# cebarker1000/heatflow

Hardware: AMD Instinct MI355X
Metric: DOF-updates/s (timesteps/s x nDOF) on geballe_with_diamond (higher is better)
Workload: dtype f64

## Files before the change

heatflow_amd/csrc/heatflow_hip.hip:

```cpp

#include "hf_amg_io.hpp"

namespace {

struct MeshTables {
  std::vector<int32_t> rowptr, colidx;
  ColDict spmv;
  RowGather rg;
  std::vector<char> tag_used;
  int max_blk_nnz = 0;
};

constexpr char BLOB_MAGIC[8] = {'H', 'F', 'P', 'A', 'T', '0', '2', 0};
struct BlobHeader {
  char magic[8];
  int64_t total_bytes, nnz;
  int32_t n, ne, rba, ts, max_blk_nnz, tab_len, rg_ok, rg_max_dict, spmv_max_dict, reserved;
  int64_t count[12];
};

void steady_swap(hf_ctx* ctx) {
  hf_ctx::Steady& S = ctx->steady;
  std::swap(ctx->nbc, S.nbc); std::swap(ctx->d_bc_dofs, S.bc_dofs); std::swap(ctx->d_g, S.g);
  std::swap(ctx->nlift_rows, S.nlift_rows); std::swap(ctx->nlift, S.nlift);
  std::swap(ctx->d_lift_rows, S.lift_rows); std::swap(ctx->d_lift_ptr, S.lift_ptr); std::swap(ctx->d_lift_bc, S.lift_bc);
  std::swap(ctx->d_lift_slot, S.lift_slot); std::swap(ctx->d_lift_val, S.lift_val);
  std::swap(ctx->d_A, S.K); std::swap(ctx->d_dinv, S.dinv);
  std::swap(ctx->amg, S.amg); std::swap(ctx->d_coarse_inv, S.coarse_inv); std::swap(ctx->d_coarse_inv_f, S.coarse_inv_f);
  std::swap(ctx->coarse_n, S.coarse_n); std::swap(ctx->coarse_ld, S.coarse_ld); std::swap(ctx->amg_ready, S.amg_ready);
  std::swap(ctx->amg_fine_stale, S.amg_fine_stale); std::swap(ctx->amg_opc, S.amg_opc); std::swap(ctx->amg_setup_s, S.amg_setup_s);
  std::swap(ctx->amg_print, S.amg_print);
}
struct SteadyScope {
  hf_ctx* c;
  explicit SteadyScope(hf_ctx* ctx) : c(ctx) { steady_swap(c); }
  ~SteadyScope() { steady_swap(c); }
  SteadyScope(const SteadyScope&) = delete;
  SteadyScope& operator=(const SteadyScope&) = delete;
};

void steady_free(hf_ctx* ctx) {
  {
    SteadyScope sw(ctx);
    free_amg(ctx);
  }
  hf_ctx::Steady& S = ctx->steady;
  dev_free(&S.bc_dofs); dev_free(&S.g); dev_free(&S.lift_rows); dev_free(&S.lift_ptr); dev_free(&S.lift_bc);
  dev_free(&S.lift_slot); dev_free(&S.lift_val); dev_free(&S.K); dev_free(&S.dinv); dev_free(&S.Kfree);
  dev_free(&S.hdr0); dev_free(&S.xprev); dev_free(&S.change);
  S.picard = false;
  S.nbc = S.nlift_rows = S.nlift = 0;
  S.ready = false;
  S.pred_iters = 0;
}

void load_free(hf_ctx* ctx) {
  dev_free(&ctx->d_load);
  ctx->have_load = false;
}

void tangent_free(hf_ctx* ctx) {
  free_batch_state(ctx->tanb);
  dev_free(&ctx->tan.col); dev_free(&ctx->tan.F);
  ctx->tan = hf_ctx::Tangent();
}

void kt_free(hf_ctx* ctx) {
  hf_ctx::KappaT& K = ctx->kt;
  dev_free(&K.hdr); dev_free(&K.vals); dev_free(&K.pic); dev_free(&K.b0); dev_free(&K.change);
  dev_free(&K.chdr); dev_free(&K.cvals); dev_free(&K.w);
  K = hf_ctx::KappaT();
}

void an_free(hf_ctx* ctx) {
  dev_free(&ctx->an.d_m);
  ctx->an = hf_ctx::Aniso();
}

const char* kt_kind(const hf_ctx* ctx) { return ctx->kt.k_on || !ctx->kt.c_on ? "kappa(T)" : "rho_c(T)"; }

int install_mesh(hf_ctx* ctx, int32_t n, int32_t ne, const double* zr, const int32_t* tri, const int32_t* tag, MeshTables& T) {
  free_batch(ctx);
  free_batch_state(ctx->fluxb);
  free_batch_cols(ctx);
  proj_free(ctx);
  steady_free(ctx);
  load_free(ctx);
  tangent_free(ctx);
  kt_free(ctx);
  an_free(ctx);
  ctx->n = n; ctx->ne = ne; ctx->nnz = static_cast<int64_t>(T.colidx.size());
  ctx->nchunks = (n + RB - 1) / RB;
  ctx->nblk_a = (n + RBA - 1) / RBA;
  ctx->P = std::min(ctx->nchunks, MAXP);
  if (ctx->P >= 64) ctx->P &= ~7;
  ctx->nchunks_s = (n + SRPC - 1) / SRPC;
  ctx->Ps = std::min(ctx->nchunks_s, MAXP);
  if (ctx->Ps >= 64) ctx->Ps &= ~7;
  ctx->max_chunk_nnz_s = 0;
  for (int c = 0; c < ctx->nchunks_s; ++c)
    ctx->max_chunk_nnz_s = std::max(ctx->max_chunk_nnz_s, T.rowptr[std::min<int64_t>(n, (c + 1LL) * SRPC)] - T.rowptr[static_cast<size_t>(c) * SRPC]);
  ctx->max_cdict = T.spmv.max_dict;
  ctx->c16 = true;
  if (const char* e = std::getenv("HEATFLOW_SPMV_C16")) ctx->c16 = (e[0] != '0');
  if (static_cast<size_t>(ctx->max_chunk_nnz_s + ctx->max_cdict) * 8 > 64 * 1024) ctx->c16 = false;
  ctx->cdict_own = static_cast<int>(T.spmv.ptr.size()) == ctx->nchunks_s + 1;
  for (int c = 0; c < ctx->nchunks_s && ctx->cdict_own; ++c) {
    const int32_t r0 = c * SRPC, r1 = std::min<int32_t>(n, r0 + SRPC);
    const int32_t* lo = T.spmv.dict.data() + T.spmv.ptr[c];
    const int32_t* hi = T.spmv.dict.data() + T.spmv.ptr[c + 1];
    const int32_t* at = std::lower_bound(lo, hi, r0);
    ctx->cdict_own = hi - at >= r1 - r0 && at[0] == r0 && at[r1 - r0 - 1] == r1 - 1;
  }
  ctx->max_blk_nnz = T.max_blk_nnz;
  if (static_cast<size_t>((ctx->max_blk_nnz + 1) & ~1) * 16 + (RBA + 1) * 4 > 160 * 1024)
    return fail(ctx, HF_ERR_ARG, "row block holds %d nonzeros: LDS slab too large", ctx->max_blk_nnz);
  ctx->tab_len = static_cast<int>(T.tag_used.size());
  ctx->h_tag_used = T.tag_used;
  ctx->assembled = false; ctx->have_mat = false;
  ctx->h_tri.assign(tri, tri + 3 * static_cast<size_t>(ne));
  ctx->h_tag.assign(tag, tag + ne);
  ctx->owner_ready = false;
  ctx->ncolors = 0; ctx->elist_len = 0;
  dev_free(&ctx->d_blk_eptr); dev_free(&ctx->d_blk_cptr); dev_free(&ctx->d_blk_ent);

  std::vector<int4> elem(ne);
  for (int32_t e = 0; e < ne; ++e) elem[e] = make_int4(tri[3 * e], tri[3 * e + 1], tri[3 * e + 2], tag[e]);
  HF_TRY(dev_alloc(ctx, &ctx->d_zr, n));
  HF_TRY(dev_alloc(ctx, &ctx->d_elem, ne));
  HF_TRY(dev_alloc(ctx, &ctx->d_kappa, ctx->tab_len));
  HF_TRY(dev_alloc(ctx, &ctx->d_rhoc, ctx->tab_len));
  HF_TRY(dev_alloc(ctx, &ctx->d_rowptr, n + 1));
  HF_TRY(dev_alloc(ctx, &ctx->d_colidx, ctx->nnz));
  HF_TRY(dev_alloc(ctx, &ctx->d_cdict_ptr, T.spmv.ptr.size()));
  HF_TRY(dev_alloc(ctx, &ctx->d_cdict, T.spmv.dict.size()));
  HF_TRY(dev_alloc(ctx, &ctx->d_cid, T.spmv.id.size()));
  ctx->n_cdict = static_cast<int64_t>(T.spmv.dict.size());
  HF_HIP(copy_sync(ctx, ctx->d_zr, zr, sizeof(double) * 2 * n, hipMemcpyHostToDevice));
  ctx->rg_ok = T.rg.ok && rowgather_smem_bytes(T.max_blk_nnz, T.rg.cols.max_dict) <= 160 * 1024;
  std::fill_n(ctx->rg_grid, static_cast<int>(RG_VARIANTS), 0);
  if (ctx->rg_ok) {
    const RowGather& G = T.rg;
    ctx->rg_max_dict = G.cols.max_dict;
    ctx->h_rg_tags = G.tags;
    ctx->n_rg_ell = static_cast<int64_t>(G.ell.size());
    ctx->n_rg_dict = static_cast<int64_t>(G.cols.dict.size());
    HF_TRY(dev_alloc(ctx, &ctx->d_rg_hdr, G.hdr.size()));
    HF_TRY(dev_alloc(ctx, &ctx->d_rg_ell, G.ell.size()));
    HF_TRY(dev_alloc(ctx, &ctx->d_rg_cid, G.cols.id.size() + 16));
    HF_TRY(dev_alloc(ctx, &ctx->d_rg_dict, G.cols.dict.size()));
    HF_TRY(dev_alloc(ctx, &ctx->d_rg_zrb, G.cols.dict.size()));
    HF_TRY(dev_alloc(ctx, &ctx->d_kappa_rg, 64));
    HF_TRY(dev_alloc(ctx, &ctx->d_rhoc_rg, 64));
    HF_HIP(copy_sync(ctx, ctx->d_rg_hdr, G.hdr.data(), sizeof(int4) * G.hdr.size(), hipMemcpyHostToDevice));
    HF_HIP(copy_sync(ctx, ctx->d_rg_ell, G.ell.data(), sizeof(uint16_t) * G.ell.size(), hipMemcpyHostToDevice));
    HF_HIP(hipMemsetAsync(ctx->d_rg_cid + G.cols.id.size(), 0, sizeof(uint16_t) * 16, ctx->stream));
    HF_HIP(copy_sync(ctx, ctx->d_rg_cid, G.cols.id.data(), sizeof(uint16_t) * G.cols.id.size(), hipMemcpyHostToDevice));
    HF_HIP(copy_sync(ctx, ctx->d_rg_dict, G.cols.dict.data(), sizeof(int32_t) * G.cols.dict.size(), hipMemcpyHostToDevice));
    const int64_t total = ctx->n_rg_dict;
    hipLaunchKernelGGL(k_gather_coords, dim3(static_cast<unsigned>((total + 255) / 256)), dim3(256), 0, ctx->stream, total, ctx->d_rg_dict,
                       ctx->d_zr, ctx->d_rg_zrb);
    HF_HIP(hipGetLastError());
  }
  HF_TRY(dev_alloc(ctx, &ctx->d_M, ctx->nnz));
  HF_TRY(dev_alloc(ctx, &ctx->d_A, ctx->nnz));
  HF_TRY(dev_alloc(ctx, &ctx->d_dinv, n));
  HF_TRY(dev_alloc(ctx, &ctx->d_u, n));
  HF_TRY(dev_alloc(ctx, &ctx->d_uprev, n));
  HF_TRY(dev_alloc(ctx, &ctx->d_ustart, n));
  ctx->have_prev = false;
  ctx->bdf_hist = false;
  free_responses(ctx);
  HF_TRY(dev_alloc(ctx, &ctx->d_b, n));
// ... 291 lines not shown
    HF_HIP(hipGetLastError());
    std::swap(ctx->batch, ctx->fluxnb);
    const int rc = batch_dispatch(ctx, [&](auto ops) { return decltype(ops)::pcg(ctx, false, rtol, 0.0, max_it); });
    int itmax = 0;
    for (int j = 0; j < nv; ++j) itmax = std::max(itmax, ctx->batch.h_scal[j].iters);
    std::swap(ctx->batch, ctx->fluxnb);
    if (it_out) it_out[done] = itmax;
    if (rc != HF_OK) { if (second) std::swap(F.u, F.uprev); return rc; }
    double* o = out + static_cast<size_t>(done) * nv * nfs;
    const int thr = nfs * nv;
    switch (nv) {
      case 2: hipLaunchKernelGGL((kb_gather<2>), dim3((thr + 255) / 256), dim3(256), 0, ctx->stream, nfs, ctx->d_fsamp_idx, F.u, o); break;
      case 4: hipLaunchKernelGGL((kb_gather<4>), dim3((thr + 255) / 256), dim3(256), 0, ctx->stream, nfs, ctx->d_fsamp_idx, F.u, o); break;
      case 8: hipLaunchKernelGGL((kb_gather<8>), dim3((thr + 255) / 256), dim3(256), 0, ctx->stream, nfs, ctx->d_fsamp_idx, F.u, o); break;
      default: hipLaunchKernelGGL((kb_gather<16>), dim3((thr + 255) / 256), dim3(256), 0, ctx->stream, nfs, ctx->d_fsamp_idx, F.u, o); break;
    }
    HF_HIP(hipGetLastError());
    if (second) std::swap(F.u, F.uprev);
    ++done;
  }
  return HF_OK;
}
int tangent_reset(hf_ctx* ctx) {
  hf_ctx::Batch& T = ctx->tanb;
  if (T.nv == 0) return HF_OK;
  HF_HIP(hipMemsetAsync(T.u, 0, sizeof(double) * static_cast<size_t>(ctx->n) * T.nv, ctx->stream));
  HF_HIP(hipStreamSynchronize(ctx->stream));
  T.bdf_hist = false;
  for (bool& u_ : T.pused) u_ = false;
  T.pnext = 0; T.ppending = -1;
  T.pred_iters = 0;
  return HF_OK;
}

int tangent_levels(hf_ctx* ctx) {
  hf_ctx::Batch& T = ctx->tanb;
  std::vector<int64_t> sig;
  if (ctx->precond == 1 && ctx->amg_ready)
    for (const DevLevel& L : ctx->amg) { sig.push_back(L.n); sig.push_back(L.P.ncol); }
  if (sig == ctx->tan.lev_sig) return HF_OK;
  for (auto& L : T.lev) { dev_free(&L.x); dev_free(&L.cat); if (L.own_b) dev_free(&L.b); }
  T.lev.clear();
  HF_TRY(batch_levels(ctx, T, T.nv));
  HF_HIP(hipStreamSynchronize(ctx->stream));
  ctx->tan.lev_sig = sig;
  return HF_OK;
}

int tangent_load(hf_ctx* ctx) {
  const int capd = ctx->rg_max_dict;
  const size_t sm = static_cast<size_t>(capd) * 16 + static_cast<size_t>(capd + (capd & 1)) * 8 + (RBA + 4) * 4 +
                    (static_cast<size_t>((ctx->max_blk_nnz + 1) & ~1) / 8 + 3) * 16;
  const int grid = std::min(ctx->nblk_a, 2048);
#define HF_TL(NV) hipLaunchKernelGGL(k_tangent_load<NV>, dim3(grid), dim3(RBA), sm, ctx->stream, ctx->nblk_a, capd, ctx->d_rg_hdr, \
                                     reinterpret_cast<const uint4*>(ctx->d_rg_ell), reinterpret_cast<const uint4*>(ctx->d_rg_cid), \
                                     ctx->d_rg_zrb, ctx->d_rg_dict, ctx->d_rowptr, ctx->tan.col, ctx->d_u, ctx->tan.F)
  switch (ctx->tan.nv) {
    case 2: HF_TL(2); break;
    case 4: HF_TL(4); break;
    case 8: HF_TL(8); break;
    default: HF_TL(16); break;
  }
#undef HF_TL
  HF_HIP(hipGetLastError());
  return HF_OK;
}

}

extern "C" {

const char* hf_version(void) { return "heatflow_hip 0.1 (gfx950)"; }

const char* hf_last_error(const hf_ctx* ctx) { return ctx ? ctx->err.c_str() : "null context"; }

int hf_create(int device_id, hf_ctx** out) {
  if (!out) return HF_ERR_ARG;
  *out = nullptr;
  int count = 0;
  if (hipGetDeviceCount(&count) != hipSuccess || count <= 0) return HF_ERR_HIP;
  if (device_id < 0 || device_id >= count) return HF_ERR_ARG;
  hf_ctx* ctx = new hf_ctx();
  ctx->dev = device_id;
  auto bail = [&](int rc) { *out = ctx; return rc; };
  if (hipSetDevice(device_id) != hipSuccess) return bail(fail(ctx, HF_ERR_HIP, "hipSetDevice(%d) failed", device_id));
  if (hipStreamCreateWithFlags(&ctx->stream, hipStreamNonBlocking) != hipSuccess)
    return bail(fail(ctx, HF_ERR_HIP, "hipStreamCreate failed"));
  if (hipEventCreate(&ctx->ev0) != hipSuccess || hipEventCreate(&ctx->ev1) != hipSuccess)
    return bail(fail(ctx, HF_ERR_HIP, "hipEventCreate failed"));
  if (hipHostMalloc(reinterpret_cast<void**>(&ctx->h_scal), sizeof(Scal)) != hipSuccess)
    return bail(fail(ctx, HF_ERR_ALLOC, "hipHostMalloc failed"));
  if (hipHostMalloc(reinterpret_cast<void**>(&ctx->h_mirror), sizeof(ScalMirror), hipHostMallocMapped | hipHostMallocCoherent) != hipSuccess ||
      hipHostGetDevicePointer(reinterpret_cast<void**>(&ctx->d_mirror), ctx->h_mirror, 0) != hipSuccess)
    return bail(fail(ctx, HF_ERR_ALLOC, "hipHostMalloc (mapped) failed"));
  *ctx->h_mirror = ScalMirror{};
  int rc = dev_alloc(ctx, &ctx->d_scal, 1);
  if (rc == HF_OK) rc = dev_alloc(ctx, &ctx->d_part_pAp, MAXP);
  if (rc == HF_OK) rc = dev_alloc(ctx, &ctx->d_part_rz, 2 * MAXP);
  if (rc == HF_OK) rc = dev_alloc(ctx, &ctx->d_part_zz, MAXP);
  if (rc == HF_OK) rc = dev_alloc(ctx, &ctx->d_part_bn, MAXP);
  if (rc == HF_OK && reset_scal(ctx) != HF_OK) rc = HF_ERR_HIP;
  if (rc == HF_OK) {
    hipLaunchKernelGGL(k_zero_entries, dim3(1), dim3(64), 0, ctx->stream, 0, static_cast<const int32_t*>(nullptr), static_cast<double*>(nullptr));
    if (hipStreamSynchronize(ctx->stream) != hipSuccess) rc = fail(ctx, HF_ERR_HIP, "first kernel launch failed: %s", hipGetErrorString(hipGetLastError()));
  }
  *out = ctx;
  return rc;
}

int hf_destroy(hf_ctx* ctx) {
  if (!ctx) return HF_ERR_ARG;
  (void)hipSetDevice(ctx->dev);
  if (ctx->stream) (void)hipStreamSynchronize(ctx->stream);
  dev_free(&ctx->d_zr); dev_free(&ctx->d_elem); dev_free(&ctx->d_kappa); dev_free(&ctx->d_rhoc);
  dev_free(&ctx->d_rowptr); dev_free(&ctx->d_colidx); dev_free(&ctx->d_cdict_ptr); dev_free(&ctx->d_cdict); dev_free(&ctx->d_cid); dev_free(&ctx->d_blk_eptr); dev_free(&ctx->d_blk_cptr); dev_free(&ctx->d_blk_ent); dev_free(&ctx->d_rg_hdr); dev_free(&ctx->d_rg_ell); dev_free(&ctx->d_rg_cid); dev_free(&ctx->d_rg_dict); dev_free(&ctx->d_rg_zrb); dev_free(&ctx->d_kappa_rg); dev_free(&ctx->d_rhoc_rg); dev_free(&ctx->d_M); dev_free(&ctx->d_A); dev_free(&ctx->d_dinv);
  dev_free(&ctx->d_bc_dofs); dev_free(&ctx->d_g); dev_free(&ctx->d_lift_rows); dev_free(&ctx->d_lift_ptr);
  dev_free(&ctx->d_lift_bc); dev_free(&ctx->d_lift_slot); dev_free(&ctx->d_lift_val);
  dev_free(&ctx->d_uprev); dev_free(&ctx->d_ustart);
  dev_free(&ctx->d_u); dev_free(&ctx->d_b); dev_free(&ctx->d_r); dev_free(&ctx->d_p); dev_free(&ctx->d_Ap);
  free_batch(ctx); free_batch_state(ctx->fluxb); free_batch_cols(ctx); free_amg(ctx); free_responses(ctx); proj_free(ctx); dev_free(&ctx->d_z); dev_free(&ctx->d_z2);
  steady_free(ctx); load_free(ctx); tangent_free(ctx); kt_free(ctx); an_free(ctx);
  dev_free(&ctx->d_M1); dev_free(&ctx->d_dinv1); dev_free(&ctx->d_gz); dev_free(&ctx->d_gr); dev_free(&ctx->d_bz); dev_free(&ctx->d_br);
  dev_free(&ctx->d_tmp); dev_free(&ctx->d_part_pAp); dev_free(&ctx->d_part_rz); dev_free(&ctx->d_part_zz);
  dev_free(&ctx->d_part_bn); dev_free(&ctx->d_scal); dev_free(&ctx->d_samp_idx); dev_free(&ctx->d_samp); dev_free(&ctx->d_fsamp_idx);
  for (auto& e : ctx->prof_ev) (void)hipEventDestroy(e);
  if (ctx->h_scal) (void)hipHostFree(ctx->h_scal);
  if (ctx->h_mirror) (void)hipHostFree(ctx->h_mirror);
  if (ctx->ev0) (void)hipEventDestroy(ctx->ev0);
  if (ctx->ev1) (void)hipEventDestroy(ctx->ev1);
  if (ctx->stream) (void)hipStreamDestroy(ctx->stream);
  delete ctx;
  return HF_OK;
}

int hf_set_mesh(hf_ctx* ctx, int32_t n, int32_t ne, const double* zr, const int32_t* tri, const int32_t* tag) {
  if (!ctx) return HF_ERR_ARG;
  if (!zr || !tri || !tag || n <= 0 || ne <= 0) return fail(ctx, HF_ERR_ARG, "hf_set_mesh: null pointer or empty mesh");
  HF_HIP(hipSetDevice(ctx->dev));
  int32_t maxtag = 0;
  for (int64_t k = 0; k < 3LL * ne; ++k)
    if (tri[k] < 0 || tri[k] >= n) return fail(ctx, HF_ERR_ARG, "hf_set_mesh: triangle %lld references node %d outside [0,%d)", (long long)(k / 3), tri[k], n);
  for (int32_t e = 0; e < ne; ++e) {
    if (tag[e] < 0) return fail(ctx, HF_ERR_ARG, "hf_set_mesh: negative cell tag at cell %d", e);
    maxtag = std::max(maxtag, tag[e]);
    const double* p0 = zr + 2 * tri[3 * e], *p1 = zr + 2 * tri[3 * e + 1], *p2 = zr + 2 * tri[3 * e + 2];
    const double d = (p1[0] - p0[0]) * (p2[1] - p0[1]) - (p2[0] - p0[0]) * (p1[1] - p0[1]);
    if (!(d != 0.0)) return fail(ctx, HF_ERR_ARG, "hf_set_mesh: degenerate triangle %d", e);
  }
  const auto t0 = std::chrono::steady_clock::now();
  auto lap = [&](const char* what) {
    if (std::getenv("HEATFLOW_DEBUG")) std::fprintf(stderr, "[set_mesh] %-28s %.3f s\n", what, std::chrono::duration<double>(std::chrono::steady_clock::now() - t0).count());
  };
  lap("checked");
  MeshTables T;
  Pattern P;
  HF_TRY(build_csr(ctx, n, ne, tri, P));
  lap("+ csr pattern");
  build_rowgather(n, ne, tri, tag, P);
  lap("+ row-gather lists");
  if (!build_coldict(P.rowptr, P.colidx, n, SRPC, T.spmv)) return fail(ctx, HF_ERR_ARG, "an SpMV chunk touches more than 65535 columns (16-bit positions)");
  lap("+ spmv column lists");
  T.rowptr.swap(P.rowptr);
  T.colidx.swap(P.colidx);
  T.max_blk_nnz = P.max_blk_nnz;
  T.rg = std::move(P.rg);
  T.tag_used.assign(static_cast<size_t>(maxtag) + 1, 0);
  for (int32_t e = 0; e < ne; ++e) T.tag_used[tag[e]] = 1;
  const int rc = install_mesh(ctx, n, ne, zr, tri, tag, T);
  lap("+ installed");
  return rc;
}

int hf_set_mesh_prebuilt(hf_ctx* ctx, int32_t n, int32_t ne, const double* zr, const int32_t* tri, const int32_t* tag,
                         const void* blob, int64_t bytes) {
  if (!ctx) return HF_ERR_ARG;
  if (!zr || !tri || !tag || !blob || n <= 0 || ne <= 0 || bytes <= 0) return fail(ctx, HF_ERR_ARG, "hf_set_mesh_prebuilt: null pointer or empty mesh");
  HF_HIP(hipSetDevice(ctx->dev));
  std::vector<unsigned char> staged;
  const unsigned char* src = nullptr;
  HF_TRY(blob_on_host(ctx, blob, bytes, staged, &src));
  MeshTables T;
  HF_TRY(parse_mesh_tables(ctx, src, bytes, n, ne, T));
  return install_mesh(ctx, n, ne, zr, tri, tag, T);
}

int hf_pattern_export_size(hf_ctx* ctx, int64_t* bytes) {
  if (!ctx || !bytes) return HF_ERR_ARG;
  if (!ctx->have_mesh) return fail(ctx, HF_ERR_STATE, "hf_pattern_export_size before hf_set_mesh");
  *bytes = mesh_tables_bytes(ctx);
  return HF_OK;
}

int hf_pattern_export(hf_ctx* ctx, void* blob, int64_t bytes) {
  if (!ctx || !blob) return HF_ERR_ARG;
  if (!ctx->have_mesh) return fail(ctx, HF_ERR_STATE, "hf_pattern_export before hf_set_mesh");
  if (bytes != mesh_tables_bytes(ctx)) return fail(ctx, HF_ERR_ARG, "hf_pattern_export: buffer of %lld bytes, need %lld", (long long)bytes, (long long)mesh_tables_bytes(ctx));
  HF_HIP(hipSetDevice(ctx->dev));
  std::vector<unsigned char> host(static_cast<size_t>(bytes));
  HF_TRY(write_mesh_tables(ctx, host.data()));
  HF_HIP(hipMemcpy(blob, host.data(), static_cast<size_t>(bytes), hipMemcpyDefault));
  return HF_OK;
}

int hf_set_materials(hf_ctx* ctx, int32_t n_mat, const int32_t* tags, const double* kappa, const double* rho_c) {
// ... 49 lines not shown
    m[q] = make_double2(by_tag[2 * tg], by_tag[2 * tg + 1]);
  }
  HF_HIP(hipSetDevice(ctx->dev));
  if (!any && !ctx->an.on) return HF_OK;
  if (any) {
    if (!ctx->an.d_m) HF_TRY(dev_alloc(ctx, &ctx->an.d_m, 64));
    HF_HIP(copy_sync(ctx, ctx->an.d_m, m.data(), sizeof(double2) * 64, hipMemcpyHostToDevice));
    ctx->an.h_tag = std::move(aniso);
    ctx->an.hash = fnv1a(by_tag.data(), sizeof(double) * by_tag.size());
    ctx->an.on = true;
  } else {
    an_free(ctx);
  }
  free_batch(ctx);
  ctx->assembled = false;
  ctx->pred_iters = 0;
  ctx->steady.ready = false;
  const bool from_steady = ctx->tan.steady_state;
  tangent_free(ctx);
  ctx->tan.steady_state = from_steady;
  return HF_OK;
}

int hf_update_kappa(hf_ctx* ctx, int32_t n_mat, const int32_t* tags, const double* kappa) {
  if (!ctx) return HF_ERR_ARG;
  if (!ctx->have_mat || !ctx->assembled) return fail(ctx, HF_ERR_STATE, "hf_update_kappa needs a completed hf_assemble first");
  if (n_mat <= 0 || !tags || !kappa) return fail(ctx, HF_ERR_ARG, "hf_update_kappa: bad arguments");
  HF_HIP(hipSetDevice(ctx->dev));
  std::vector<double> tk(ctx->tab_len);
  HF_HIP(copy_sync(ctx, tk.data(), ctx->d_kappa, sizeof(double) * ctx->tab_len, hipMemcpyDeviceToHost));
  for (int32_t i = 0; i < n_mat; ++i) {
    if (tags[i] < 0 || tags[i] >= ctx->tab_len || !ctx->h_tag_used[tags[i]])
      return fail(ctx, HF_ERR_ARG, "hf_update_kappa: tag %d is not a cell tag of the mesh", tags[i]);
    if (!(kappa[i] > 0.0)) return fail(ctx, HF_ERR_ARG, "hf_update_kappa: kappa must be positive");
    if (ctx->kt.k_on && ctx->kt.tabled[tags[i]])
      return fail(ctx, HF_ERR_ARG, "hf_update_kappa: tag %d carries a kappa(T) table (hf_set_kappa_tables)", tags[i]);
  }
  for (int32_t i = 0; i < n_mat; ++i) {
    tk[tags[i]] = kappa[i];
  }
  HF_HIP(copy_sync(ctx, ctx->d_kappa, tk.data(), sizeof(double) * ctx->tab_len, hipMemcpyHostToDevice));
  HF_TRY(upload_rg_tables(ctx, tk, nullptr));
  ctx->steady.ready = false;
  return hf_assemble(ctx, ctx->dt_step, ctx->mode);
}

int hf_set_dirichlet(hf_ctx* ctx, int32_t n_bc, const int32_t* dofs) {
  if (!ctx) return HF_ERR_ARG;
  if (!ctx->have_mesh) return fail(ctx, HF_ERR_STATE, "hf_set_dirichlet before hf_set_mesh");
  if (n_bc < 0 || (n_bc > 0 && !dofs)) return fail(ctx, HF_ERR_ARG, "hf_set_dirichlet: bad arguments");
  HF_HIP(hipSetDevice(ctx->dev));
  std::vector<char> seen(ctx->n, 0);
  for (int32_t q = 0; q < n_bc; ++q) {
    if (dofs[q] < 0 || dofs[q] >= ctx->n) return fail(ctx, HF_ERR_ARG, "hf_set_dirichlet: dof %d outside [0,%d)", dofs[q], ctx->n);
    if (seen[dofs[q]]) return fail(ctx, HF_ERR_ARG, "hf_set_dirichlet: dof %d listed twice (resolve overlaps on the host)", dofs[q]);
    seen[dofs[q]] = 1;
  }
  free_batch(ctx);
  ctx->nbc = n_bc;
  HF_TRY(dev_alloc(ctx, &ctx->d_bc_dofs, n_bc));
  HF_TRY(dev_alloc(ctx, &ctx->d_g, n_bc));
  if (n_bc > 0) HF_HIP(copy_sync(ctx, ctx->d_bc_dofs, dofs, sizeof(int32_t) * n_bc, hipMemcpyHostToDevice));
  HF_TRY(build_lift(ctx));
  free_amg(ctx);
  free_responses(ctx);
  ctx->assembled = false;
  return HF_OK;
}

int hf_assemble(hf_ctx* ctx, double dt, int32_t mode) {
  if (!ctx) return HF_ERR_ARG;
  if (!ctx->have_mesh || !ctx->have_mat) return fail(ctx, HF_ERR_STATE, "hf_assemble needs hf_set_mesh and hf_set_materials first");
  if (!(dt > 0.0)) return fail(ctx, HF_ERR_ARG, "hf_assemble: dt must be positive");
  if (mode < 0 || mode > 3) return fail(ctx, HF_ERR_ARG, "hf_assemble: unknown mode %d", mode);
  if (ctx->kt.on && mode != HF_ASM_ROW_GATHER)
    return fail(ctx, HF_ERR_ARG, "hf_assemble: %s tables are evaluated by the row-gather kernel only (HF_ASM_ROW_GATHER)", kt_kind(ctx));
  if (ctx->an.on && (mode != HF_ASM_ROW_GATHER || !ctx->rg_ok))
    return fail(ctx, HF_ERR_ARG, "hf_assemble: anisotropic conductivities (hf_set_anisotropy) are assembled by the row-gather kernel only (HF_ASM_ROW_GATHER)");
  HF_HIP(hipSetDevice(ctx->dev));
  ctx->dt_step = dt;
  ctx->dt = ctx->scheme == HF_TIME_BDF2 ? 2.0 * dt / 3.0 : dt;
  ctx->mode = mode;
  HF_HIP(hipEventRecord(ctx->ev0, ctx->stream));
  HF_TRY(launch_assemble(ctx));
  if (ctx->kt.on) {
    HF_TRY(kt_revalue(ctx, ctx->d_u, nullptr));
  } else {
    if (ctx->nbc > 0) {
      if (ctx->nlift > 0)
        hipLaunchKernelGGL(k_take_lift, dim3((ctx->nlift + 255) / 256), dim3(256), 0, ctx->stream, ctx->nlift,
                           ctx->d_lift_slot, ctx->d_A, ctx->d_lift_val);
      hipLaunchKernelGGL(k_bc_rows, dim3((ctx->nbc + 255) / 256), dim3(256), 0, ctx->stream, ctx->nbc, ctx->d_bc_dofs,
                         ctx->d_rowptr, ctx->d_colidx, ctx->d_A);
    }
    hipLaunchKernelGGL(k_dinv, dim3((ctx->n + 255) / 256), dim3(256), 0, ctx->stream, ctx->n, ctx->d_rowptr,
                       ctx->d_colidx, ctx->d_A, ctx->d_dinv);
  }
  HF_HIP(hipEventRecord(ctx->ev1, ctx->stream));
  HF_HIP(hipGetLastError());
  HF_HIP(hipStreamSynchronize(ctx->stream));
  float ms = 0.f;
  HF_HIP(hipEventElapsedTime(&ms, ctx->ev0, ctx->ev1));
  ctx->last_ms = ms;
  if (ctx->precond == 1) {
    OperatorPrint now;
    HF_TRY(operator_print(ctx, now));
    if (!(ctx->amg_ready && ctx->amg_reuse)) {
      HF_TRY(build_amg_auto(ctx));
      ctx->amg_print = std::move(now);
    } else {
      ctx->amg_fine_stale = !same_print(now, ctx->amg_print) || ctx->kt.on;
    }
  }
  if (ctx->precond == 1 && ctx->amg_ready) {
    ctx->amg[0].A.val = ctx->d_A;
    ctx->amg[0].dinv = ctx->d_dinv;
  }
  ctx->assembled = true;
  ctx->pred_iters = 0;
  ctx->have_prev = false;
  ctx->bdf_hist = false;
  free_responses(ctx);
  return tangent_reset(ctx);
}

int hf_set_precond(hf_ctx* ctx, int32_t kind, int32_t reuse) {
  if (!ctx) return HF_ERR_ARG;
  if (kind < 0 || kind > 1) return fail(ctx, HF_ERR_ARG, "hf_set_precond: unknown preconditioner %d", kind);
  if (kind != ctx->precond) { ctx->assembled = false; ctx->pred_iters = 0; (void)hipSetDevice(ctx->dev); free_batch(ctx); }
  if (kind == 0) { (void)hipSetDevice(ctx->dev); free_amg(ctx); }
  ctx->precond = kind;
  ctx->amg_reuse = reuse ? 1 : 0;
  return HF_OK;
}

int hf_set_time_scheme(hf_ctx* ctx, int32_t scheme) {
  if (!ctx) return HF_ERR_ARG;
  if (scheme != HF_TIME_BACKWARD_EULER && scheme != HF_TIME_BDF2) return fail(ctx, HF_ERR_ARG, "hf_set_time_scheme: unknown scheme %d", scheme);
  if (scheme != ctx->scheme) {
    (void)hipSetDevice(ctx->dev);
    free_batch(ctx);
    ctx->assembled = false;
    ctx->pred_iters = 0;
    ctx->scheme = scheme;
  }
  return HF_OK;
}

int kt_set_tables(hf_ctx* ctx, bool cap, int32_t n_tab, const int32_t* tags, const double* t0, const double* dT, const int32_t* n_knots,
                  const double* values) {
  const char* fn = cap ? "hf_set_rhoc_tables" : "hf_set_kappa_tables";
  const char* what = cap ? "rho_c(T)" : "kappa(T)";
  if (!ctx) return HF_ERR_ARG;
  if (!ctx->have_mesh) return fail(ctx, HF_ERR_STATE, "%s before hf_set_mesh", fn);
  if (n_tab < 0) return fail(ctx, HF_ERR_ARG, "%s: negative table count", fn);
  HF_HIP(hipSetDevice(ctx->dev));
  hf_ctx::KappaT& K = ctx->kt;
  if (n_tab == 0) {
    if (ctx->steady.picard) ctx->steady.ready = false;
    if (cap ? K.c_on : K.k_on) {
      free_batch(ctx);
      ctx->assembled = false;
      ctx->pred_iters = 0;
    }
    if (!(cap ? K.k_on : K.c_on)) { kt_free(ctx); return HF_OK; }
    if (cap ? K.c_on : K.k_on) {
      const std::vector<KTab> none(64, KTab{0.0, 0.0, 0, 0});
      HF_HIP(copy_sync(ctx, cap ? K.chdr : K.hdr, none.data(), sizeof(KTab) * 64, hipMemcpyHostToDevice));
      dev_free(cap ? &K.cvals : &K.vals);
      (cap ? K.ctabled : K.tabled).clear();
      (cap ? K.c_on : K.k_on) = false;
      K.have_change = false;
    }
    return HF_OK;
  }
  if (!tags || !t0 || !dT || !n_knots || !values) return fail(ctx, HF_ERR_ARG, "%s: null pointer", fn);
  if (ctx->an.on) return fail(ctx, HF_ERR_STATE, "%s: anisotropic conductivities are set (hf_set_anisotropy; the table kernels are isotropic)", fn);
  if (!ctx->rg_ok || (ctx->assembled && ctx->mode != HF_ASM_ROW_GATHER))
    return fail(ctx, HF_ERR_ARG, "%s: %s is evaluated by the row-gather kernel only (HF_ASM_ROW_GATHER on a mesh with row-gather lists)", fn, what);
  if (cap && ct_smem_bytes(ctx->max_blk_nnz, ctx->rg_max_dict) + 2 * 64 * sizeof(KTab) > 160 * 1024)
    return fail(ctx, HF_ERR_ARG, "%s: the (M, A) slab, the staged state and the table headers of this mesh exceed the 160 KiB of LDS", fn);
  std::vector<KTab> hdr(64, KTab{0.0, 0.0, 0, 0});
  std::vector<double> vals;
  std::vector<char> tabled(ctx->tab_len, 0);
  for (int32_t i = 0; i < n_tab; ++i) {
    const int32_t tg = tags[i];
// ... 437 lines not shown
  if (ctx->have_load) return fail(ctx, HF_ERR_STATE, "hf_run_tangent: a load is set (tangents of pre-heated runs are not supported)");
  if (!ctx->tan.ready) return fail(ctx, HF_ERR_STATE, "hf_run_tangent before hf_tangent_setup");
  if (ctx->tan.steady_state)
    return fail(ctx, HF_ERR_STATE, "hf_run_tangent: the state comes from hf_steady_solve and depends on the conductivities (tangents start at zero): hf_set_state first");
  if (!ctx->assembled) return fail(ctx, HF_ERR_STATE, "hf_run_tangent before hf_assemble");
  if (ctx->mode != HF_ASM_ROW_GATHER) return fail(ctx, HF_ERR_ARG, "hf_run_tangent: the operator was not assembled by the row-gather kernel");
  if (n_steps <= 0 || (ctx->nbc > 0 && !g_all) || max_it <= 0 || rtol < 0 || atol < 0) return fail(ctx, HF_ERR_ARG, "hf_run_tangent: bad arguments");
  if (ns < 0 || (ns > 0 && (!nodes || !samples || !tangent_samples))) return fail(ctx, HF_ERR_ARG, "hf_run_tangent: bad sample arguments");
  for (int32_t q = 0; q < ns; ++q)
    if (nodes[q] < 0 || nodes[q] >= ctx->n) return fail(ctx, HF_ERR_ARG, "hf_run_tangent: node %d outside [0,%d)", nodes[q], ctx->n);
  HF_HIP(hipSetDevice(ctx->dev));
  hf_ctx::Batch& T = ctx->tanb;
  const int nv = T.nv;
  const size_t hstep = static_cast<size_t>(ctx->nbc) * nv;
  DevTemp<double> t_gall, t_hall, t_sall, t_tall;
  if (ctx->nbc > 0) {
    HF_TRY(dev_alloc(ctx, &t_gall.p, static_cast<size_t>(n_steps) * ctx->nbc));
    HF_HIP(copy_sync(ctx, t_gall.p, g_all, sizeof(double) * n_steps * ctx->nbc, hipMemcpyHostToDevice));
    HF_TRY(dev_alloc(ctx, &t_hall.p, h_all ? hstep * n_steps : hstep));
    if (h_all) HF_HIP(copy_sync(ctx, t_hall.p, h_all, sizeof(double) * hstep * n_steps, hipMemcpyHostToDevice));
    else HF_HIP(hipMemsetAsync(t_hall.p, 0, sizeof(double) * hstep, ctx->stream));
  }
  if (ns > 0) {
    HF_TRY(ensure_samples(ctx, ns));
    HF_TRY(dev_alloc(ctx, &t_sall.p, static_cast<size_t>(n_steps) * ns));
    HF_TRY(dev_alloc(ctx, &t_tall.p, static_cast<size_t>(n_steps) * nv * ns));
    HF_HIP(copy_sync(ctx, ctx->d_samp_idx, nodes, sizeof(int32_t) * ns, hipMemcpyHostToDevice));
  }
  HF_TRY(ensure_batch_cols(ctx, nv));
  T.lds = ctx->bcols.nv == nv;
  HF_TRY(tangent_levels(ctx));
  int rc = HF_OK;
  HF_HIP(hipEventRecord(ctx->ev0, ctx->stream));
  for (int32_t s = 0; s < n_steps && rc == HF_OK; ++s) {
    rc = step_device(ctx, ctx->nbc > 0 ? g_all + static_cast<size_t>(s) * ctx->nbc : nullptr,
                     ctx->nbc > 0 ? t_gall.p + static_cast<size_t>(s) * ctx->nbc : nullptr, rtol, atol, max_it);
    if (iters) iters[s] = ctx->h_scal->iters;
    if (rc != HF_OK) break;
    if (ns > 0)
      hipLaunchKernelGGL(k_gather, dim3((ns + 255) / 256), dim3(256), 0, ctx->stream, ns, ctx->d_samp_idx, ctx->d_u,
                         t_sall.p + static_cast<size_t>(s) * ns);
    HF_TRY(tangent_load(ctx));
    const double* hs = ctx->nbc == 0 ? nullptr : t_hall.p + (h_all ? hstep * s : 0);
    std::swap(ctx->batch, ctx->tanb);
    rc = batch_dispatch(ctx, [&](auto ops) { return decltype(ops)::step(ctx, hs, rtol, atol, max_it); });
    std::swap(ctx->batch, ctx->tanb);
    if (tangent_iters)
      for (int j = 0; j < nv; ++j) tangent_iters[static_cast<size_t>(s) * nv + j] = T.h_scal[j].iters;
    if (ns > 0 && rc == HF_OK) {
      double* out = t_tall.p + static_cast<size_t>(s) * nv * ns;
      const int thr = ns * nv;
      switch (nv) {
        case 2: hipLaunchKernelGGL((kb_gather<2>), dim3((thr + 255) / 256), dim3(256), 0, ctx->stream, ns, ctx->d_samp_idx, T.u, out); break;
        case 4: hipLaunchKernelGGL((kb_gather<4>), dim3((thr + 255) / 256), dim3(256), 0, ctx->stream, ns, ctx->d_samp_idx, T.u, out); break;
        case 8: hipLaunchKernelGGL((kb_gather<8>), dim3((thr + 255) / 256), dim3(256), 0, ctx->stream, ns, ctx->d_samp_idx, T.u, out); break;
        default: hipLaunchKernelGGL((kb_gather<16>), dim3((thr + 255) / 256), dim3(256), 0, ctx->stream, ns, ctx->d_samp_idx, T.u, out); break;
      }
    }
  }
  (void)hipEventRecord(ctx->ev1, ctx->stream);
  (void)hipStreamSynchronize(ctx->stream);
  float ms = 0.f;
  (void)hipEventElapsedTime(&ms, ctx->ev0, ctx->ev1);
  ctx->last_ms = ms;
  if (ns > 0 && rc == HF_OK) {
    (void)copy_sync(ctx, samples, t_sall.p, sizeof(double) * n_steps * ns, hipMemcpyDeviceToHost);
    (void)copy_sync(ctx, tangent_samples, t_tall.p, sizeof(double) * n_steps * nv * ns, hipMemcpyDeviceToHost);
  }
  return rc;
}

int hf_get_tangent(hf_ctx* ctx, int32_t j, double* s) {
  if (!ctx) return HF_ERR_ARG;
  if (!ctx->tan.ready) return fail(ctx, HF_ERR_STATE, "hf_get_tangent before hf_tangent_setup");
  if (j < 0 || j >= ctx->tan.nv || !s) return fail(ctx, HF_ERR_ARG, "hf_get_tangent: column %d outside [0,%d) or null pointer", j, ctx->tan.nv);
  HF_HIP(hipSetDevice(ctx->dev));
  hipLaunchKernelGGL(kb_get_column, dim3(1024), dim3(256), 0, ctx->stream, static_cast<size_t>(ctx->n), ctx->tan.nv, j, ctx->tanb.u, ctx->d_tmp);
  HF_HIP(hipGetLastError());
  HF_HIP(copy_sync(ctx, s, ctx->d_tmp, sizeof(double) * ctx->n, hipMemcpyDeviceToHost));
  return HF_OK;
}

int steady_eliminate(hf_ctx* ctx) {
  HF_HIP(hipMemcpyAsync(ctx->d_A, ctx->steady.Kfree, sizeof(double) * ctx->nnz, hipMemcpyDeviceToDevice, ctx->stream));
  if (ctx->nlift > 0)
    hipLaunchKernelGGL(k_take_lift, dim3((ctx->nlift + 255) / 256), dim3(256), 0, ctx->stream, ctx->nlift, ctx->d_lift_slot,
                       ctx->d_A, ctx->d_lift_val);
  hipLaunchKernelGGL(k_bc_rows, dim3((ctx->nbc + 255) / 256), dim3(256), 0, ctx->stream, ctx->nbc, ctx->d_bc_dofs, ctx->d_rowptr,
                     ctx->d_colidx, ctx->d_A);
  hipLaunchKernelGGL(k_dinv, dim3((ctx->n + 255) / 256), dim3(256), 0, ctx->stream, ctx->n, ctx->d_rowptr, ctx->d_colidx, ctx->d_A, ctx->d_dinv);
  HF_HIP(hipGetLastError());
  return HF_OK;
}

int steady_setup_impl(hf_ctx* ctx, const char* fn, bool picard, int32_t n_s, const int32_t* dofs, int32_t precond) {
  if (n_s <= 0 || !dofs) return fail(ctx, HF_ERR_ARG, "%s: empty Dirichlet set (the stiffness alone is singular)", fn);
  if (precond < 0 || precond > 1) return fail(ctx, HF_ERR_ARG, "%s: unknown preconditioner %d", fn, precond);
  if (!ctx->rg_ok || (ctx->assembled && ctx->mode != HF_ASM_ROW_GATHER))
    return fail(ctx, HF_ERR_ARG, "%s: the steady operator is assembled by the row-gather kernel only (HF_ASM_ROW_GATHER on a mesh with row-gather lists)", fn);
  std::vector<char> seen(ctx->n, 0);
  for (int32_t q = 0; q < n_s; ++q) {
    if (dofs[q] < 0 || dofs[q] >= ctx->n) return fail(ctx, HF_ERR_ARG, "%s: dof %d outside [0,%d)", fn, dofs[q], ctx->n);
    if (seen[dofs[q]]) return fail(ctx, HF_ERR_ARG, "%s: dof %d listed twice (resolve overlaps on the host)", fn, dofs[q]);
    seen[dofs[q]] = 1;
  }
  HF_HIP(hipSetDevice(ctx->dev));
  steady_free(ctx);
  hf_ctx::Steady& S = ctx->steady;
  const int n = ctx->n;
  S.nbc = n_s;
  HF_TRY(dev_alloc(ctx, &S.bc_dofs, n_s));
  HF_TRY(dev_alloc(ctx, &S.g, n_s));
  HF_TRY(dev_alloc(ctx, &S.Kfree, ctx->nnz));
  HF_TRY(dev_alloc(ctx, &S.K, ctx->nnz));
  HF_TRY(dev_alloc(ctx, &S.dinv, n));
  if (picard) {
    HF_TRY(dev_alloc(ctx, &S.xprev, n));
    HF_TRY(dev_alloc(ctx, &S.change, 1));
    if (!ctx->kt.hdr) {
      const std::vector<KTab> none(64, KTab{0.0, 0.0, 0, 0});
      HF_TRY(dev_alloc(ctx, &S.hdr0, 64));
      HF_HIP(copy_sync(ctx, S.hdr0, none.data(), sizeof(KTab) * 64, hipMemcpyHostToDevice));
    }
  }
  HF_HIP(copy_sync(ctx, S.bc_dofs, dofs, sizeof(int32_t) * n_s, hipMemcpyHostToDevice));
  HF_HIP(hipEventRecord(ctx->ev0, ctx->stream));
  if (picard) HF_TRY(steady_revalue(ctx, ctx->kt.hdr ? ctx->kt.hdr : S.hdr0, ctx->d_u, S.Kfree));
  else HF_TRY(launch_assemble_rows_any<true>(ctx, ctx->d_kappa_rg, ctx->d_rhoc_rg, 1.0, nullptr, S.Kfree));
  {
    SteadyScope sw(ctx);
    HF_TRY(build_lift(ctx));
    HF_TRY(steady_eliminate(ctx));
    HF_HIP(hipEventRecord(ctx->ev1, ctx->stream));
    HF_HIP(hipGetLastError());
    HF_HIP(hipStreamSynchronize(ctx->stream));
    float ms = 0.f;
    HF_HIP(hipEventElapsedTime(&ms, ctx->ev0, ctx->ev1));
    ctx->last_ms = ms;
    if (precond == 1) HF_TRY(build_amg_auto(ctx));
  }
  S.precond = precond;
  S.pred_iters = 0;
  S.picard = picard;
  S.ready = true;
  return HF_OK;
}

int hf_steady_setup(hf_ctx* ctx, int32_t n_s, const int32_t* dofs, int32_t precond) {
  if (!ctx) return HF_ERR_ARG;
  if (!ctx->have_mesh || !ctx->have_mat) return fail(ctx, HF_ERR_STATE, "hf_steady_setup needs hf_set_mesh and hf_set_materials first");
  if (ctx->kt.on) return fail(ctx, HF_ERR_STATE, "hf_steady_setup: %s tables are set (a Picard steady state is not supported)", kt_kind(ctx));
  return steady_setup_impl(ctx, "hf_steady_setup", false, n_s, dofs, precond);
}

int hf_steady_picard_setup(hf_ctx* ctx, int32_t n_s, const int32_t* dofs, int32_t precond) {
  if (!ctx) return HF_ERR_ARG;
  if (!ctx->have_mesh || !ctx->have_mat) return fail(ctx, HF_ERR_STATE, "hf_steady_picard_setup needs hf_set_mesh and hf_set_materials first");
  if (ctx->an.on)
    return fail(ctx, HF_ERR_STATE, "hf_steady_picard_setup: anisotropic conductivities are set (hf_set_anisotropy; the table kernels are isotropic)");
  return steady_setup_impl(ctx, "hf_steady_picard_setup", true, n_s, dofs, precond);
}

int hf_steady_picard_solve(hf_ctx* ctx, const double* g_s, int32_t use_load, double rtol, double atol, int32_t max_it, double picard_tol,
                           int32_t max_sweeps, int32_t* sweeps, int32_t* iters, double* change, double* nl_resid) {
  if (!ctx) return HF_ERR_ARG;
  if (!ctx->steady.ready || !ctx->steady.picard)
// ... 341 lines not shown
  for (int32_t q = 0; q < ns; ++q)
    if (nodes[q] < 0 || nodes[q] >= ctx->n) return fail(ctx, HF_ERR_ARG, "hf_batch_run: node %d outside [0,%d)", nodes[q], ctx->n);
  const int ncomp = (flux_components & 1) + ((flux_components >> 1) & 1);
  if (flux_components != 0) {
    if (flux_components < 0 || flux_components > 3 || flux_max_it <= 0 || flux_rtol < 0 || nfs <= 0 || !flux_nodes || !flux_samples)
      return fail(ctx, HF_ERR_ARG, "hf_batch_run_flux: bad flux arguments");
    if (!ctx->flux_ready) return fail(ctx, HF_ERR_STATE, "hf_batch_run_flux before hf_flux_setup");
    if (!ctx->rg_ok) return fail(ctx, HF_ERR_ARG, "hf_batch_run_flux: the row-gather lists are not available for this mesh (a row of more than 32 entries or more than 64 cell tags): project run by run");
    for (int32_t q = 0; q < nfs; ++q)
      if (flux_nodes[q] < 0 || flux_nodes[q] >= ctx->n) return fail(ctx, HF_ERR_ARG, "hf_batch_run_flux: node %d outside [0,%d)", flux_nodes[q], ctx->n);
  }
  HF_HIP(hipSetDevice(ctx->dev));
  const int nv = B.nv;
  const size_t gstep = static_cast<size_t>(ctx->nbc) * nv;
  DevTemp<double> t_sall, t_fall;
  if (flux_components != 0) {
    HF_TRY(ensure_batch_flux(ctx, nv, ncomp));
    if (nfs > ctx->fsamp_cap) { HF_TRY(dev_alloc(ctx, &ctx->d_fsamp_idx, nfs)); ctx->fsamp_cap = nfs; }
    HF_HIP(copy_sync(ctx, ctx->d_fsamp_idx, flux_nodes, sizeof(int32_t) * nfs, hipMemcpyHostToDevice));
    HF_TRY(dev_alloc(ctx, &t_fall.p, static_cast<size_t>(n_steps) * ncomp * nv * nfs));
  }
  if (ctx->nbc > 0) {
    HF_TRY(dev_alloc(ctx, &B.g, gstep * n_steps));
    HF_HIP(copy_sync(ctx, B.g, g_all, sizeof(double) * gstep * n_steps, hipMemcpyHostToDevice));
  }
  if (ns > 0) {
    HF_TRY(ensure_samples(ctx, ns));
    HF_TRY(dev_alloc(ctx, &t_sall.p, static_cast<size_t>(n_steps) * nv * ns));
    HF_HIP(copy_sync(ctx, ctx->d_samp_idx, nodes, sizeof(int32_t) * ns, hipMemcpyHostToDevice));
  }
  int rc = HF_OK;
  HF_HIP(hipEventRecord(ctx->ev0, ctx->stream));
  for (int32_t s = 0; s < n_steps && rc == HF_OK; ++s) {
    const double* gs = ctx->nbc > 0 ? B.g + gstep * s : nullptr;
    rc = batch_dispatch(ctx, [&](auto ops) { return decltype(ops)::step(ctx, gs, rtol, atol, max_it); });
    if (iters)
      for (int j = 0; j < nv; ++j) iters[static_cast<size_t>(s) * nv + j] = B.h_scal[j].iters;
    if (ns > 0 && rc == HF_OK) {
      double* out = t_sall.p + static_cast<size_t>(s) * nv * ns;
      const int thr = ns * nv;
      switch (nv) {
        case 2: hipLaunchKernelGGL((kb_gather<2>), dim3((thr + 255) / 256), dim3(256), 0, ctx->stream, ns, ctx->d_samp_idx, B.u, out); break;
        case 4: hipLaunchKernelGGL((kb_gather<4>), dim3((thr + 255) / 256), dim3(256), 0, ctx->stream, ns, ctx->d_samp_idx, B.u, out); break;
        case 8: hipLaunchKernelGGL((kb_gather<8>), dim3((thr + 255) / 256), dim3(256), 0, ctx->stream, ns, ctx->d_samp_idx, B.u, out); break;
        default: hipLaunchKernelGGL((kb_gather<16>), dim3((thr + 255) / 256), dim3(256), 0, ctx->stream, ns, ctx->d_samp_idx, B.u, out); break;
      }
    }
    if (flux_components != 0 && rc == HF_OK)
      rc = batch_flux_step(ctx, flux_components, flux_rtol, flux_max_it, nfs, t_fall.p + static_cast<size_t>(s) * ncomp * nv * nfs,
                           flux_iters ? flux_iters + static_cast<size_t>(s) * ncomp : nullptr);
  }
  (void)hipEventRecord(ctx->ev1, ctx->stream);
  (void)hipStreamSynchronize(ctx->stream);
  float ms = 0.f;
  (void)hipEventElapsedTime(&ms, ctx->ev0, ctx->ev1);
  ctx->last_ms = ms;
  if (ns > 0 && rc == HF_OK) (void)copy_sync(ctx, samples, t_sall.p, sizeof(double) * n_steps * nv * ns, hipMemcpyDeviceToHost);
  if (flux_components != 0 && rc == HF_OK)
    (void)copy_sync(ctx, flux_samples, t_fall.p, sizeof(double) * n_steps * ncomp * nv * nfs, hipMemcpyDeviceToHost);
  return rc;
}

int hf_get_sizes(hf_ctx* ctx, int32_t* n, int32_t* ne, int64_t* nnz, int32_t* nbc) {
  if (!ctx) return HF_ERR_ARG;
  if (n) *n = ctx->n;
  if (ne) *ne = ctx->ne;
  if (nnz) *nnz = ctx->nnz;
  if (nbc) *nbc = ctx->nbc;
  return HF_OK;
}

int hf_get_csr(hf_ctx* ctx, int32_t* rowptr, int32_t* colidx, double* A, double* M) {
  if (!ctx) return HF_ERR_ARG;
  if (!ctx->have_mesh) return fail(ctx, HF_ERR_STATE, "hf_get_csr before hf_set_mesh");
  if ((A || M) && !ctx->assembled) return fail(ctx, HF_ERR_STATE, "hf_get_csr: values requested before hf_assemble");
  HF_HIP(hipSetDevice(ctx->dev));
  if (rowptr) std::memcpy(rowptr, ctx->h_rowptr.data(), sizeof(int32_t) * (ctx->n + 1));
  if (colidx) std::memcpy(colidx, ctx->h_colidx.data(), sizeof(int32_t) * ctx->nnz);
  if (A) HF_HIP(copy_sync(ctx, A, ctx->d_A, sizeof(double) * ctx->nnz, hipMemcpyDeviceToHost));
  if (M) HF_HIP(copy_sync(ctx, M, ctx->d_M, sizeof(double) * ctx->nnz, hipMemcpyDeviceToHost));
  return HF_OK;
}

int hf_spmv(hf_ctx* ctx, int32_t which, const double* x, double* y) {
  if (!ctx) return HF_ERR_ARG;
  if (!ctx->assembled || !x || !y || which < 0 || which > 1) return fail(ctx, HF_ERR_STATE, "hf_spmv: not assembled or bad arguments");
  HF_HIP(hipSetDevice(ctx->dev));
  HF_HIP(copy_sync(ctx, ctx->d_tmp, x, sizeof(double) * ctx->n, hipMemcpyHostToDevice));
  launch_spmv<0>(ctx, which ? ctx->d_M : ctx->d_A, ctx->d_tmp, ctx->d_Ap);
  HF_HIP(hipGetLastError());
  HF_HIP(hipStreamSynchronize(ctx->stream));
  HF_HIP(copy_sync(ctx, y, ctx->d_Ap, sizeof(double) * ctx->n, hipMemcpyDeviceToHost));
  return HF_OK;
}

int hf_amg_apply(hf_ctx* ctx, const double* r, double* z, double* rz) {
  if (!ctx || !r || !z) return HF_ERR_ARG;
  if (ctx->precond != 1 || !ctx->amg_ready || !ctx->assembled || ctx->amg.empty())
    return fail(ctx, HF_ERR_STATE, "hf_amg_apply: no assembled operator with a multigrid hierarchy (hf_set_precond(1, ...) and hf_assemble first)");
  HF_HIP(hipSetDevice(ctx->dev));
  const int n = ctx->n, nl = static_cast<int>(ctx->amg.size());
  HF_TRY(reset_scal(ctx));
  std::vector<double> dinv(n), z0(n);
  HF_HIP(copy_sync(ctx, dinv.data(), ctx->d_dinv, sizeof(double) * n, hipMemcpyDeviceToHost));
  const double w0 = ctx->amg[0].omega;
  for (int i = 0; i < n; ++i) z0[i] = w0 * (dinv[i] * r[i]);
  auto poison = [&](double* p, size_t count) { return count ? hipMemsetAsync(p, 0xFF, sizeof(double) * count, ctx->stream) : hipSuccess; };
  HF_HIP(poison(ctx->d_tmp, n));
  HF_HIP(poison(ctx->d_z2, n));
  HF_HIP(poison(ctx->d_part_rz, MAXP));
  for (int l = 1; l < nl; ++l) {
    DevLevel& L = ctx->amg[l];
    if (L.cat) HF_HIP(poison(L.cat, static_cast<size_t>(L.n) + ctx->amg[l + 1].n));
    else HF_HIP(poison(L.b, L.n));
    if (l == 1) HF_HIP(poison(L.res, L.n));
  }
  HF_HIP(copy_sync(ctx, ctx->d_r, r, sizeof(double) * n, hipMemcpyHostToDevice));
  HF_HIP(copy_sync(ctx, ctx->d_z, z0.data(), sizeof(double) * n, hipMemcpyHostToDevice));
  vcycle(ctx, 0);
  HF_HIP(hipGetLastError());
  HF_HIP(hipStreamSynchronize(ctx->stream));
  HF_HIP(copy_sync(ctx, z, ctx->d_z2, sizeof(double) * n, hipMemcpyDeviceToHost));
  if (rz) {
    std::vector<double> part(ctx->P);
    HF_HIP(copy_sync(ctx, part.data(), ctx->d_part_rz, sizeof(double) * ctx->P, hipMemcpyDeviceToHost));
    double s = 0.0;
    for (double v : part) s += v;
    *rz = s;
  }
  return HF_OK;
}

int hf_batch_apply_precond(hf_ctx* ctx, const double* r, double* z, double* rz) {
  if (!ctx || !r || !z) return HF_ERR_ARG;
  hf_ctx::Batch& B = ctx->batch;
  if (B.nv == 0) return fail(ctx, HF_ERR_STATE, "hf_batch_apply_precond: no batch is open (hf_batch_begin)");
  if (ctx->precond != 1 || !ctx->amg_ready || !ctx->assembled || ctx->amg.empty() || B.lev.size() != ctx->amg.size())
    return fail(ctx, HF_ERR_STATE, "hf_batch_apply_precond: the batch has no multigrid hierarchy");
  HF_HIP(hipSetDevice(ctx->dev));
  const int nv = B.nv, nl = static_cast<int>(ctx->amg.size());
  const size_t n = static_cast<size_t>(ctx->n), vec = n * nv;
  const bool dpc = B.opk != HF_BATCH_SHARED;
  std::vector<double> dinv(dpc ? vec : n), ri(vec), z0(vec);
  HF_HIP(copy_sync(ctx, dinv.data(), dpc ? B.dinv : ctx->d_dinv, sizeof(double) * dinv.size(), hipMemcpyDeviceToHost));
  const double w0 = ctx->amg[0].omega;
  for (size_t i = 0; i < n; ++i)
    for (int j = 0; j < nv; ++j) {
      const size_t q = i * nv + j;
      ri[q] = r[static_cast<size_t>(j) * n + i];
      z0[q] = w0 * ((dpc ? dinv[q] : dinv[i]) * ri[q]);
    }
  auto poison = [&](double* p, size_t count) { return count ? hipMemsetAsync(p, 0xFF, sizeof(double) * count, ctx->stream) : hipSuccess; };
  HF_HIP(poison(B.tmp, vec));
  HF_HIP(poison(B.z2, vec));
  HF_HIP(poison(B.part_rz, static_cast<size_t>(nv) * MAXP));
  for (int l = 1; l < nl; ++l) {
    const hf_ctx::BatchLevel& Q = B.lev[l];
    const size_t ln = static_cast<size_t>(ctx->amg[l].n);
    if (Q.cat) HF_HIP(poison(Q.cat, (ln + ctx->amg[l + 1].n) * nv));
    else HF_HIP(poison(Q.b, ln * nv));
    if (l == 1) HF_HIP(poison(Q.res, ln * nv));
  }
  HF_HIP(hipMemsetAsync(B.scal, 0, sizeof(Scal) * nv, ctx->stream));
  HF_HIP(copy_sync(ctx, B.r, ri.data(), sizeof(double) * vec, hipMemcpyHostToDevice));
  HF_HIP(copy_sync(ctx, B.z, z0.data(), sizeof(double) * vec, hipMemcpyHostToDevice));
  HF_TRY(batch_dispatch(ctx, [&](auto ops) { decltype(ops)::vcycle(ctx, 0); return HF_OK; }));
// ... 151 lines not shown
```

heatflow_amd/csrc/hf_context.hpp:

```cpp

#pragma once
#include <hip/hip_runtime.h>
#include <hip/hip_ext.h>

#include <algorithm>
#include <chrono>
#include <cmath>
#include <cstdarg>
#include <cstdint>
#include <cstdio>
#include <cstdlib>
#include <cstring>
#include <string>
#include <thread>
#include <vector>

#include "amg_host.hpp"
#include "heatflow_hip.h"

namespace {

constexpr int RB = 256;
#ifndef HF_RBA
#define HF_RBA 256
#endif
constexpr int RBA = HF_RBA;
constexpr int TPB = 256;
constexpr int NCOL = 32;
#ifndef HF_STAGE_U
#define HF_STAGE_U 2
#endif
#ifndef HF_UNROLL
#define HF_UNROLL 4
#endif
constexpr int MAXP = 1024;
constexpr int MAXRESP = 4;
#ifndef HF_PROJ_MH
#define HF_PROJ_MH 6
#endif
constexpr int PROJ_MH = HF_PROJ_MH;
constexpr int PROJ_MT = PROJ_MH + MAXRESP;
constexpr int TS = 512;
#ifndef HF_SPMV_RPC
#define HF_SPMV_RPC 512
#endif
#ifndef HF_SPMV_UN
#define HF_SPMV_UN 8
#endif
constexpr int SRPC = HF_SPMV_RPC;

struct ScalMirror {
  double zz, bn2;
  int iters;
  int pad_;
  unsigned long long done_st;
  unsigned long long tested_st;
};
inline int mirror_tested(const ScalMirror* m, unsigned epoch) {
  const unsigned long long v = __atomic_load_n(&m->tested_st, __ATOMIC_ACQUIRE);
  return static_cast<unsigned>(v >> 32) == epoch ? static_cast<int>(v & 0xffffffffu) - 1 : -1;
}
inline int mirror_done(const ScalMirror* m, unsigned epoch) {
  const unsigned long long v = __atomic_load_n(&m->done_st, __ATOMIC_ACQUIRE);
  return static_cast<unsigned>(v >> 32) == epoch ? static_cast<int>(v & 0xffffffffu) : 0;
}

struct Scal {
  double tol2;
  double bn2;
  double zz;
  int iters;
  int done;
  int first;
  unsigned epoch;
  ScalMirror* mirror;
};

constexpr int NV_MAX = 16;
struct BRed { double pAp[NV_MAX], rz[2][NV_MAX], zz[NV_MAX], bn[NV_MAX]; };

constexpr int KT_MAX_KNOTS = 256;
constexpr int KT_MAX_PICARD = 8;
struct KTab { double t0, inv_dt; int n, off; };

enum RgVariant { RG_ROWS, RG_ROWS_K, RG_AN, RG_AN_K, RG_KT, RG_CT, RG_KT_K, RG_VARIANTS };

}

struct hf_ctx {
  int dev = 0;
  hipStream_t stream = nullptr;
  hipEvent_t ev0 = nullptr, ev1 = nullptr;
  std::string err;
  double last_ms = 0.0;

  int32_t n = 0, ne = 0, nbc = 0;
  int64_t nnz = 0;
  int nchunks = 0, P = 0;
  int nchunks_s = 0, Ps = 0;
  int max_chunk_nnz_s = 0;
  int32_t *d_cdict_ptr = nullptr, *d_cdict = nullptr;
  uint16_t* d_cid = nullptr;
  int max_cdict = 0;
  bool cdict_own = false;
  bool c16 = true;
  bool have_mesh = false, have_mat = false, assembled = false;
  double dt = 0.0;
  double dt_step = 0.0;
  int mode = 0;
  int scheme = HF_TIME_BACKWARD_EULER;

  std::vector<int32_t> h_rowptr, h_colidx, h_tri, h_tag;
  std::vector<char> h_tag_used;
  bool owner_ready = false;

  double2* d_zr = nullptr;
  int4* d_elem = nullptr;
  int tab_len = 0;
  double *d_kappa = nullptr, *d_rhoc = nullptr;
  int32_t *d_rowptr = nullptr, *d_colidx = nullptr;
  int32_t *d_blk_eptr = nullptr, *d_blk_cptr = nullptr;
  int2* d_blk_ent = nullptr;
  int nblk_a = 0;
  int max_blk_nnz = 0, ncolors = 0;
  int64_t elist_len = 0;
  bool rg_ok = false;
  int4* d_rg_hdr = nullptr;
  uint16_t *d_rg_ell = nullptr, *d_rg_cid = nullptr;
  int32_t* d_rg_dict = nullptr;
  double2* d_rg_zrb = nullptr;
  int rg_max_dict = 0;
  int rg_grid[RG_VARIANTS] = {};
  int64_t n_rg_ell = 0, n_rg_dict = 0, n_cdict = 0;
  std::vector<int32_t> h_rg_tags;
  double *d_kappa_rg = nullptr, *d_rhoc_rg = nullptr;
  struct Aniso {
    bool on = false;
    double2* d_m = nullptr;
    std::vector<char> h_tag;
    uint64_t hash = 0;
  } an;
  double *d_M = nullptr, *d_A = nullptr, *d_dinv = nullptr;
  int32_t* d_bc_dofs = nullptr;
  double* d_g = nullptr;
  int32_t nlift_rows = 0, nlift = 0;
  int32_t *d_lift_rows = nullptr, *d_lift_ptr = nullptr, *d_lift_bc = nullptr, *d_lift_slot = nullptr;
  double* d_lift_val = nullptr;
  double *d_u = nullptr, *d_b = nullptr, *d_r = nullptr, *d_p = nullptr, *d_Ap = nullptr;
  double *d_uprev = nullptr, *d_ustart = nullptr;
  bool have_prev = false;
  bool bdf_hist = false;
  int extrapolate = 1;
  int start_kind = 3;
  std::vector<double> h_g0, h_g1;
  int g_hist = 0;
  struct BcResponse { std::vector<double> dir; double* w = nullptr; };
  std::vector<BcResponse> resp;
  long long resp_solves = 0;
  struct Proj {
    double *V[PROJ_MT] = {nullptr}, *F[PROJ_MT] = {nullptr};
    bool used[PROJ_MT] = {false};
    int next = 0, pending = -1;
    double *G = nullptr, *alpha = nullptr, *part = nullptr;
    bool ready = false;
  } proj;
  double *d_tmp = nullptr;
  double *d_part_pAp = nullptr, *d_part_rz = nullptr, *d_part_zz = nullptr, *d_part_bn = nullptr;
  Scal* d_scal = nullptr;
  Scal* h_scal = nullptr;
  ScalMirror* h_mirror = nullptr;
  ScalMirror* d_mirror = nullptr;
  unsigned epoch = 0;
  int32_t* d_samp_idx = nullptr;
  double* d_samp = nullptr;
  int samp_cap = 0;
  int pred_iters = 0;
  int precond = 0;
  int amg_reuse = 0;
  bool amg_ready = false;
  struct DevCsr {
    int nrow = 0, ncol = 0, lanes = 8; int64_t nnz = 0; int32_t *ptr = nullptr, *idx = nullptr; double* val = nullptr;
    float* valf = nullptr;
    int max_row = 0;
    int rpc = 0, nchunks = 0, chunk_nnz = 0;
    int32_t *dptr = nullptr, *dict = nullptr;
    uint16_t* cid = nullptr;
    int max_dict = 0;
    int64_t ndict = 0;
// ... 173 lines not shown
```

heatflow_amd/csrc/hf_kernels.hpp:

```cpp
#pragma once
#include <type_traits>

#include "hf_context.hpp"

namespace {


template <int NW = 4>
__device__ __forceinline__ double block_sum(double v, double* sw) {
#pragma unroll
  for (int o = 32; o > 0; o >>= 1) v += __shfl_down(v, o, 64);
  const int w = threadIdx.x >> 6;
  if ((threadIdx.x & 63) == 0) sw[w] = v;
  __syncthreads();
  double t = sw[0];
#pragma unroll
  for (int k = 1; k < NW; ++k) t += sw[k];
  __syncthreads();
  return t;
}

__device__ __forceinline__ double sum_partials(const double* __restrict__ part, int P, double* s4) {
  double v = 0.0;
  for (int k = threadIdx.x; k < P; k += TPB) v += part[k];
// ... 701 lines not shown

__global__ void k_take_lift(int nlift, const int32_t* __restrict__ slot, double* __restrict__ A,
                            double* __restrict__ val) {
  const int q = blockIdx.x * blockDim.x + threadIdx.x;
  if (q >= nlift) return;
  val[q] = A[slot[q]];
  A[slot[q]] = 0.0;
}

__global__ void k_bc_rows(int nbc, const int32_t* __restrict__ dofs, const int32_t* __restrict__ rowptr,
                          const int32_t* __restrict__ colidx, double* __restrict__ A) {
  const int q = blockIdx.x * blockDim.x + threadIdx.x;
  if (q >= nbc) return;
  const int row = dofs[q];
  for (int k = rowptr[row]; k < rowptr[row + 1]; ++k) A[k] = (colidx[k] == row) ? 1.0 : 0.0;
}

__global__ void k_dinv(int n, const int32_t* __restrict__ rowptr, const int32_t* __restrict__ colidx,
                       const double* __restrict__ A, double* __restrict__ dinv) {
  const int row = blockIdx.x * blockDim.x + threadIdx.x;
  if (row >= n) return;
  double d = 0.0;
  for (int k = rowptr[row]; k < rowptr[row + 1]; ++k)
    if (colidx[k] == row) d = A[k];
  dinv[row] = 1.0 / d;
}

__global__ void k_lift(int nrows, const int32_t* __restrict__ rows, const int32_t* __restrict__ ptr,
                       const int32_t* __restrict__ bc, const double* __restrict__ val,
                       const double* __restrict__ g, double* __restrict__ b) {
  const int q = blockIdx.x * blockDim.x + threadIdx.x;
  if (q >= nrows) return;
  double s = 0.0;
  for (int k = ptr[q]; k < ptr[q + 1]; ++k) s += val[k] * g[bc[k]];
  b[rows[q]] -= s;
}

__global__ void k_set_bc(int nbc, const int32_t* __restrict__ dofs, const double* __restrict__ g,
                         double* __restrict__ b, double* __restrict__ u) {
  const int q = blockIdx.x * blockDim.x + threadIdx.x;
  if (q >= nbc) return;
  b[dofs[q]] = g[q];
  u[dofs[q]] = g[q];
}

__global__ void k_gather(int ns, const int32_t* __restrict__ idx, const double* __restrict__ u,
                         double* __restrict__ out) {
  const int q = blockIdx.x * blockDim.x + threadIdx.x;
  if (q < ns) out[q] = u[idx[q]];
}

__global__ __launch_bounds__(TPB) void k_hold_load(int n, const int32_t* __restrict__ rowptr, const int32_t* __restrict__ colidx,
                                                   const double* __restrict__ K, const double* __restrict__ u,
                                                   const unsigned char* __restrict__ mask, double* __restrict__ F) {
  const int row = blockIdx.x * blockDim.x + threadIdx.x;
  if (row >= n) return;
  double s = 0.0;
  if (!mask[row])
    for (int k = rowptr[row]; k < rowptr[row + 1]; ++k) s += K[k] * u[colidx[k]];
  F[row] = s;
}

__global__ void k_mark_rows(int nq, const int32_t* __restrict__ idx, unsigned char* __restrict__ mask) {
  const int q = blockIdx.x * blockDim.x + threadIdx.x;
  if (q < nq) mask[idx[q]] = 1;
}

__device__ __forceinline__ unsigned long long mirror_stamp(unsigned epoch, int v) {
  return (static_cast<unsigned long long>(epoch) << 32) | static_cast<unsigned>(v);
}
__device__ __forceinline__ void mirror_publish(ScalMirror* m, double zz, int iters, int done, unsigned epoch) {
  if (m == nullptr) return;
  m->zz = zz;
  m->iters = iters;
  __hip_atomic_store(&m->done_st, mirror_stamp(epoch, done), __ATOMIC_RELAXED, __HIP_MEMORY_SCOPE_SYSTEM);
  __threadfence_system();
  __hip_atomic_store(&m->tested_st, mirror_stamp(epoch, iters + 1), __ATOMIC_RELEASE, __HIP_MEMORY_SCOPE_SYSTEM);
}
__device__ __forceinline__ void mirror_breakdown(ScalMirror* m, unsigned epoch) {
  if (m != nullptr) __hip_atomic_store(&m->done_st, mirror_stamp(epoch, 2), __ATOMIC_RELEASE, __HIP_MEMORY_SCOPE_SYSTEM);
}

struct ColComp { const int32_t* dptr; const int32_t* dict; const uint16_t* id; int xd_off; int own; };

#ifndef HF_NT_STREAM
#define HF_NT_STREAM 0
#endif
#ifndef HF_PIPE
#define HF_PIPE 1
#endif
#ifndef HF_PHASE_CLOCK
#define HF_PHASE_CLOCK -1
#endif
#if HF_PHASE_CLOCK >= 0
#ifndef HF_PHASE_CONV
#define HF_PHASE_CONV 0
#endif
__device__ unsigned long long g_phase[MAXP * 16];
#define HF_STAMP(slot)                                                                                   \
  do {                                                                                                   \
    if (MODE == HF_PHASE_CLOCK && C16 && (MODE != 0 || (part2 != nullptr) == (HF_PHASE_CONV != 0)) && threadIdx.x == 0 && (slot) < 16) \
      g_phase[blockIdx.x * 16 + (slot)] = wall_clock64();                                                \
  } while (0)
#else
#define HF_STAMP(slot) do { } while (0)
#endif
template <typename T>
__device__ __forceinline__ T stream_load(const T* p) {
#if HF_NT_STREAM
  return __builtin_nontemporal_load(p);
#else
  return *p;
#endif
}

__device__ __forceinline__ double bdf2_operand(double un, double unm1) { return (4.0 * un - unm1) * (1.0 / 3.0); }

template <int MODE, bool C16 = false, typename VT = double, int UN = 8>
__global__ __launch_bounds__(TS) __attribute__((amdgpu_waves_per_eu(8, 8))) void k_spmv(int n, int nchunks, int rpc ,
                                              const int32_t* __restrict__ rowptr, const int32_t* __restrict__ colidx,
                                              const VT* __restrict__ vals, const double* __restrict__ x,
                                              double* __restrict__ y, Scal* __restrict__ scal,
                                              double* __restrict__ part0, const double* __restrict__ bvec,
                                              const double* __restrict__ dinv, double* __restrict__ pvec,
                                              double* __restrict__ part1, double* __restrict__ part2, double w,
                                              int npart ,
                                              int parity, ColComp comp) {
  extern __shared__ double sprod[];
  __shared__ double s4[TS / 64];
  __shared__ int s_own;
  constexpr bool BDF = MODE >= 12 && MODE <= 15;
  auto opnd = [&](int c) { return BDF ? bdf2_operand(x[c], bvec[c]) : x[c]; };
  if ((MODE == 3 || MODE == 4 || MODE == 6 || MODE == 9) && scal->done) return;
  if ((MODE == 0 || MODE == 7) && scal != nullptr && scal->done) return;
  double acc0 = 0.0, acc1 = 0.0, acc2 = 0.0;
  double beta = 0.0;
  bool first9 = false;
  if (MODE == 9) {
    first9 = scal->first != 0;
    if (!first9) {
      double v0 = 0.0, v1 = 0.0, v2 = 0.0;
      for (int k = threadIdx.x; k < npart; k += TS) {
        v0 += part1[parity * MAXP + k];
        v1 += part1[(parity ^ 1) * MAXP + k];
        v2 += part2[k];
      }
      const double rz_new = block_sum<TS / 64>(v0, s4);
      const double rz_old = block_sum<TS / 64>(v1, s4);
      const double zz = block_sum<TS / 64>(v2, s4);
      const bool conv = zz <= scal->tol2;
      if (blockIdx.x == 0 && threadIdx.x == 0) {
        scal->zz = zz;
        if (conv) scal->done = 1;
      }
      if (conv) return;
      beta = rz_new / rz_old;
    }
  }
  auto cycle_gate = [&]() {
    if (!((MODE == 3 || MODE == 0) && part2 != nullptr)) return false;
    double v2 = 0.0;
    for (int k = threadIdx.x; k < npart; k += TS) v2 += part2[k];
    const double zz = block_sum<TS / 64>(v2, s4);
    const bool conv = zz <= scal->tol2;
    if (blockIdx.x == 0 && threadIdx.x == 0) {
      if (conv) { scal->zz = zz; scal->done = 1; }
      mirror_publish(scal->mirror, zz, scal->iters, conv ? 1 : 0, scal->epoch);
    }
    return conv;
  };
  constexpr bool PIPELINED = C16 && (HF_PIPE == 2 || (HF_PIPE == 1 && sizeof(VT) == 4));
  if (!PIPELINED && cycle_gate()) return;
  const ChunkIter sched(nchunks);
  HF_STAMP(0);
  int stamp_at = 1;
  (void)stamp_at;
  const int tpr = (MODE == 0 || MODE == 6 || MODE == 7) ? TS / rpc : 1;
  const int prel = static_cast<int>(threadIdx.x) / tpr;
  const int psub = static_cast<int>(threadIdx.x) % tpr;
  struct RowOps { double b, d, y, p, x; };
  auto row_operands = [&](int prc, bool from_slice) {
    RowOps e{0.0, 0.0, 0.0, 0.0, 0.0};
    if (MODE == 2 || MODE == 3 || MODE == 4 || MODE == 5 || MODE == 7 || MODE == 8 || MODE == 11 || MODE == 13 || MODE == 15) e.b = bvec[prc];
    if (MODE == 2 || MODE == 4 || MODE == 5 || MODE == 10 || MODE == 11 || MODE == 14 || MODE == 15) e.d = dinv[prc];
    if (MODE == 6 || (MODE == 9 && !first9)) e.y = y[prc];
    if (MODE == 9 && !first9) e.p = pvec[prc];
    if ((MODE == 4 || MODE == 8 || MODE == 9 || MODE == 11) && !from_slice) e.x = x[prc];
    if (BDF) e.x = x[prc];
    return e;
  };
  auto rows_phase = [&](bool pin, int prow, int pa, int pb, const RowOps& e) {
    if ((MODE == 0 || MODE == 6 || MODE == 7) && tpr > 1) {
      double s = 0.0;
      if (pin)
        for (int j = pa + psub; j < pb; j += tpr) s += sprod[j];
      for (int o = tpr >> 1; o > 0; o >>= 1) s += __shfl_down(s, o, 64);
      if (pin && psub == 0) {
        y[prow] = (MODE == 6) ? e.y + s : s;
        if (MODE == 7) acc0 += e.b * s;
      }
    } else if (pin) {
      const int row = prow;
      double s = 0.0;
      for (int j = pa; j < pb; ++j) s += sprod[j];
      if (MODE == 0) {
        y[row] = s;
      } else if (MODE == 2) {
        const double ri = e.b - s;
        const double zi = e.d * ri;
        y[row] = ri;
        pvec[row] = zi;
        acc0 += ri * zi;
        acc1 += zi * zi;
        acc2 += (e.d * e.b) * (e.d * e.b);
      } else if (MODE == 3) {
        y[row] = e.b - s;
      } else if (MODE == 4) {
        const double yi = e.x + w * e.d * (e.b - s);
        y[row] = yi;
        acc0 += e.b * yi;
      } else if (MODE == 5) {
        const double ri = e.b - s;
        y[row] = ri;
        pvec[row] = w * e.d * ri;
        acc1 += (e.d * ri) * (e.d * ri);
        acc2 += (e.d * e.b) * (e.d * e.b);
      } else if (MODE == 7) {
        y[row] = s;
        acc0 += e.b * s;
      } else if (MODE == 6) {
        y[row] = e.y + s;
      } else if (MODE == 8) {
        y[row] = s;
        pvec[row] = 2.0 * e.x - e.b;
      } else if (MODE == 10) {
        y[row] = s + w * e.d;
      } else if (MODE == 11) {
        y[row] = s + w * e.d;
        pvec[row] = 2.0 * e.x - e.b;
      } else if (BDF) {
        y[row] = (MODE == 14 || MODE == 15) ? s + w * e.d : s;
        pvec[row] = (MODE == 13 || MODE == 15) ? 2.0 * e.x - e.b : e.x;
      } else {
        const double api = first9 ? s : s + beta * e.y;
        const double pi = first9 ? e.x : e.x + beta * e.p;
        y[row] = api;
        pvec[row] = pi;
        acc0 += pi * api;
      }
    }
  };
  if (PIPELINED) {
    struct Bounds { int k0, k1, d0, d1; };
    auto bounds = [&](int ch) {
// ... 23 lines not shown
    Bounds cur = bounds(min(sched.chunk, nchunks - 1));
    heads(cur, sched.chunk < sched.end);
    if (cycle_gate()) return;
    for (int chunk = sched.chunk; chunk < sched.end; chunk += sched.step) {
      const bool more = chunk + sched.step < sched.end;
      const int r0 = chunk * rpc, r1 = min(n, r0 + rpc);
      const int k0 = cur.k0, k1 = cur.k1, d0 = cur.d0, nd = cur.d1 - cur.d0;
      const int prow = r0 + prel;
      const bool pin = prow < r1;
      const int prc = min(prow, r1 - 1);
      int c0[HF_STAGE_U];
      double x0[HF_STAGE_U];
#pragma unroll
      for (int u = 0; u < HF_STAGE_U; ++u) { c0[u] = lhead[u]; x0[u] = opnd(c0[u]); }
      const Bounds nxt = bounds(more ? chunk + sched.step : chunk);
      const int pa = rowptr[prc] - k0, pb = rowptr[prc + 1] - k0;
      RowOps e = row_operands(prc, comp.own != 0);
#pragma unroll
      for (int u = 0; u < HF_STAGE_U; ++u) {
        const int i = static_cast<int>(threadIdx.x) + u * TS;
        if (i < nd) {
          xd[i] = x0[u];
          if ((MODE == 4 || MODE == 8 || MODE == 9 || MODE == 11) && c0[u] == r0) s_own = i;
        }
      }
      for (int i = threadIdx.x + HF_STAGE_U * TS; i < nd; i += HF_STAGE_U * TS) {
        int c[HF_STAGE_U];
        double xv[HF_STAGE_U];
#pragma unroll
        for (int u = 0; u < HF_STAGE_U; ++u) c[u] = comp.dict[d0 + min(i + u * TS, nd - 1)];
#pragma unroll
        for (int u = 0; u < HF_STAGE_U; ++u) xv[u] = opnd(c[u]);
#pragma unroll
        for (int u = 0; u < HF_STAGE_U; ++u)
          if (i + u * TS < nd) {
            xd[i + u * TS] = xv[u];
            if ((MODE == 4 || MODE == 8 || MODE == 9 || MODE == 11) && c[u] == r0) s_own = i + u * TS;
          }
      }
      __syncthreads();
      HF_STAMP(stamp_at); ++stamp_at;
      if ((MODE == 4 || MODE == 8 || MODE == 9 || MODE == 11) && comp.own && pin) e.x = xd[s_own + (prow - r0)];
#pragma unroll
      for (int u = 0; u < UN; ++u) {
        const int kk = k0 + static_cast<int>(threadIdx.x) + u * TS;
        if (kk < k1) sprod[kk - k0] = v[u] * xd[id[u]];
      }
      for (int kb = k0 + UN * TS; kb < k1; kb += UN * TS) {
#pragma unroll
        for (int u = 0; u < UN; ++u) {
          const int kk = min(kb + static_cast<int>(threadIdx.x) + u * TS, k1 - 1);
          v[u] = static_cast<double>(stream_load(&vals[kk]));
          id[u] = static_cast<int>(stream_load(&comp.id[kk]));
        }
#pragma unroll
        for (int u = 0; u < UN; ++u) {
          const int kk = kb + static_cast<int>(threadIdx.x) + u * TS;
          if (kk < k1) sprod[kk - k0] = v[u] * xd[id[u]];
        }
      }
      heads(nxt, more);
      __syncthreads();
      HF_STAMP(stamp_at); ++stamp_at;
      rows_phase(pin, prow, pa, pb, e);
      __syncthreads();
      HF_STAMP(stamp_at); ++stamp_at;
      cur = nxt;
    }
  } else {
  const ChunkIter& sched_ = sched;
  for (int chunk = sched_.chunk; chunk < sched_.end; chunk += sched_.step) {
    const int r0 = chunk * rpc;
    const int r1 = min(n, r0 + rpc);
    const int k0 = rowptr[r0];
    const int k1 = rowptr[r1];
    const int prow = r0 + prel;
    const bool pin = prow < r1;
    int pa = 0, pb = 0;
    if (pin) {
      pa = rowptr[prow] - k0;
      pb = rowptr[prow + 1] - k0;
    }
    RowOps e = row_operands(min(prow, r1 - 1), C16 && comp.own != 0);
    if (C16) {
      double* xd = sprod + comp.xd_off;
      const int d0 = comp.dptr[chunk], nd = comp.dptr[chunk + 1] - d0;
      int k = k0 + threadIdx.x;
      double v[HF_UNROLL];
      int id[HF_UNROLL];
#pragma unroll
      for (int u = 0; u < HF_UNROLL; ++u) {
        const bool in = k + u * TS < k1;
        v[u] = in ? static_cast<double>(stream_load(&vals[k + u * TS])) : 0.0;
        id[u] = in ? static_cast<int>(stream_load(&comp.id[k + u * TS])) : 0;
      }
      for (int i = threadIdx.x; i < nd; i += HF_STAGE_U * TS) {
        int c[HF_STAGE_U];
        double xv[HF_STAGE_U];
#pragma unroll
        for (int u = 0; u < HF_STAGE_U; ++u) c[u] = (i + u * TS < nd) ? comp.dict[d0 + i + u * TS] : 0;
#pragma unroll
        for (int u = 0; u < HF_STAGE_U; ++u) xv[u] = (i + u * TS < nd) ? opnd(c[u]) : 0.0;
#pragma unroll
        for (int u = 0; u < HF_STAGE_U; ++u)
          if (i + u * TS < nd) {
            xd[i + u * TS] = xv[u];
            if ((MODE == 4 || MODE == 8 || MODE == 9 || MODE == 11) && c[u] == r0) s_own = i + u * TS;
          }
      }
      __syncthreads();
      HF_STAMP(stamp_at); ++stamp_at;
      if ((MODE == 4 || MODE == 8 || MODE == 9 || MODE == 11) && comp.own && pin) e.x = xd[s_own + (prow - r0)];
      while (k < k1) {
        const int kn = k + HF_UNROLL * TS;
        double vn[HF_UNROLL];
        int idn[HF_UNROLL];
#pragma unroll
        for (int u = 0; u < HF_UNROLL; ++u) {
          const bool in = kn + u * TS < k1;
          vn[u] = in ? static_cast<double>(stream_load(&vals[kn + u * TS])) : 0.0;
          idn[u] = in ? static_cast<int>(stream_load(&comp.id[kn + u * TS])) : 0;
        }
#pragma unroll
        for (int u = 0; u < HF_UNROLL; ++u)
          if (k + u * TS < k1) sprod[k - k0 + u * TS] = v[u] * xd[id[u]];
#pragma unroll
        for (int u = 0; u < HF_UNROLL; ++u) { v[u] = vn[u]; id[u] = idn[u]; }
        k = kn;
      }
    } else {
      for (int k = k0 + threadIdx.x; k < k1; k += HF_UNROLL * TS) {
        int c[HF_UNROLL];
        double v[HF_UNROLL], xv[HF_UNROLL];
#pragma unroll
        for (int u = 0; u < HF_UNROLL; ++u) {
          const bool in = k + u * TS < k1;
          c[u] = in ? colidx[k + u * TS] : 0;
          v[u] = in ? static_cast<double>(vals[k + u * TS]) : 0.0;
        }
#pragma unroll
        for (int u = 0; u < HF_UNROLL; ++u) xv[u] = (k + u * TS < k1) ? opnd(c[u]) : 0.0;
#pragma unroll
        for (int u = 0; u < HF_UNROLL; ++u)
          if (k + u * TS < k1) sprod[k - k0 + u * TS] = v[u] * xv[u];
      }
    }
    __syncthreads();
    HF_STAMP(stamp_at); ++stamp_at;
    rows_phase(pin, prow, pa, pb, e);
    __syncthreads();
    HF_STAMP(stamp_at); ++stamp_at;
  }
  }
  if (MODE == 2 || MODE == 7 || MODE == 9 || (MODE == 4 && part0 != nullptr)) {
    const double t0 = block_sum<TS / 64>(acc0, s4);
    if (threadIdx.x == 0) {
      part0[blockIdx.x] = t0;
      for (int q = blockIdx.x + gridDim.x; q < npart; q += gridDim.x) part0[q] = 0.0;
    }
  }
  if (MODE == 2 || MODE == 5) {
    const double t1 = block_sum<TS / 64>(acc1, s4);
    const double t2 = block_sum<TS / 64>(acc2, s4);
    if (threadIdx.x == 0) {
      part1[blockIdx.x] = t1;
      part2[blockIdx.x] = t2;
      for (int q = blockIdx.x + gridDim.x; q < npart; q += gridDim.x) { part1[q] = 0.0; part2[q] = 0.0; }
    }
  }
}

__global__ __launch_bounds__(TPB) void k_pcg_begin(int P, double rtol, double atol, const double* __restrict__ part_zz,
                                                   const double* __restrict__ part_bn, Scal* __restrict__ scal, unsigned epoch) {
  __shared__ double s4[4];
  const double zz = sum_partials(part_zz, P, s4);
  const double bn2 = sum_partials(part_bn, P, s4);
  if (threadIdx.x == 0) {
    const double tol = fmax(rtol * sqrt(bn2 > 0.0 ? bn2 : zz), atol);
    scal->tol2 = tol * tol;
    scal->bn2 = bn2;
    scal->zz = zz;
    scal->iters = 0;
    scal->first = 1;
    scal->done = (zz <= tol * tol) ? 1 : 0;
    scal->epoch = epoch;
    if (scal->mirror != nullptr) scal->mirror->bn2 = bn2;
    mirror_publish(scal->mirror, zz, 0, scal->done, epoch);
  }
}

__global__ __launch_bounds__(TPB) void k_pcg_update(int n, int nchunks, int P, int parity, Scal* __restrict__ scal,
                                                    const double* __restrict__ part_pAp, double* __restrict__ part_rz,
                                                    double* __restrict__ part_zz, double* __restrict__ x,
                                                    double* __restrict__ r, const double* __restrict__ p,
                                                    const double* __restrict__ Ap, const double* __restrict__ dinv,
                                                    double* __restrict__ z) {
  __shared__ double s4[4];
  if (scal->done) return;
  const double pAp = sum_partials(part_pAp, P, s4);
  const double rz = sum_partials(part_rz + parity * MAXP, P, s4);
  if (!(pAp > 0.0)) {
    if (blockIdx.x == 0 && threadIdx.x == 0) {
      scal->done = 2;
      mirror_breakdown(scal->mirror, scal->epoch);
    }
    return;
  }
  if (blockIdx.x == 0 && threadIdx.x == 0) { scal->iters += 1; scal->first = 0; }
  const double alpha = rz / pAp;
  double a_rz = 0.0, a_zz = 0.0;
  const ChunkIter sched(nchunks);
  for (int chunk = sched.chunk; chunk < sched.end; chunk += sched.step) {
    const int i = chunk * RB + threadIdx.x;
    if (i < n) {
      const double ri = r[i] - alpha * Ap[i];
      const double zi = dinv[i] * ri;
      x[i] += alpha * p[i];
      r[i] = ri;
      z[i] = zi;
      a_rz += ri * zi;
      a_zz += zi * zi;
    }
  }
  const double t0 = block_sum(a_rz, s4);
  const double t1 = block_sum(a_zz, s4);
  if (threadIdx.x == 0) {
    part_rz[(parity ^ 1) * MAXP + blockIdx.x] = t0;
    part_zz[blockIdx.x] = t1;
  }
}

template <int LANES, int VMODE, typename VT = double>
__global__ __launch_bounds__(TPB) void k_spmv_vec(int nrow, const int32_t* __restrict__ ptr,
                                                  const int32_t* __restrict__ idx, const VT* __restrict__ val,
                                                  const double* __restrict__ x, double* __restrict__ y,
                                                  const Scal* __restrict__ scal) {
  if (scal->done) return;
  const int lane = threadIdx.x % LANES;
  const int rows_per_pass = (gridDim.x * TPB) / LANES;
  for (int row = (blockIdx.x * TPB + threadIdx.x) / LANES; row < nrow; row += rows_per_pass) {
    const int k1 = ptr[row + 1];
    const double y0 = (VMODE == 1 && lane == 0) ? y[row] : 0.0;
    double s = 0.0;
    for (int k = ptr[row] + lane; k < k1; k += 4 * LANES) {
      int c[4];
      double v[4], xv[4];
#pragma unroll
      for (int u = 0; u < 4; ++u) {
        const bool in = k + u * LANES < k1;
        c[u] = in ? idx[k + u * LANES] : 0;
        v[u] = in ? static_cast<double>(val[k + u * LANES]) : 0.0;
// ... 447 lines not shown
```

heatflow_amd/csrc/hf_pattern.hpp:

```cpp
#pragma once
#include <thread>

#include "hf_kernels.hpp"

namespace {

struct ColDict {
  std::vector<int32_t> ptr, dict;
  std::vector<uint16_t> id;
  int max_dict = 0;
};

struct RowGather {
  bool ok = false;
  std::vector<int4> hdr;
  std::vector<uint16_t> ell;
  std::vector<int32_t> tags;
  ColDict cols;
};

struct OwnerLists {
  std::vector<int32_t> blk_eptr, blk_cptr, blk_elist;
  std::vector<int2> blk_ent;
  int ncolors = 0;
// ... 290 lines not shown
                               hipFuncAttributeMaxDynamicSharedMemorySize, static_cast<int>(sm)));
  }
  if (colored)
    hipLaunchKernelGGL(k_assemble_lds<true>, dim3(ctx->nblk_a), dim3(RBA), sm, ctx->stream, ctx->n, cap, ctx->d_rowptr,
                       ctx->d_blk_eptr, ctx->d_blk_cptr, ctx->d_blk_ent, ctx->d_zr, kappa_tab, rhoc_tab, dt, Mout, Aout);
  else
    hipLaunchKernelGGL(k_assemble_lds<false>, dim3(ctx->nblk_a), dim3(RBA), sm, ctx->stream, ctx->n, cap, ctx->d_rowptr,
                       ctx->d_blk_eptr, ctx->d_blk_cptr, ctx->d_blk_ent, ctx->d_zr, kappa_tab, rhoc_tab, dt, Mout, Aout);
  HF_HIP(hipGetLastError());
  return HF_OK;
}

size_t rowgather_lds_bytes(int max_blk_nnz, int max_dict, bool pair, bool state) {
  const size_t cap = static_cast<size_t>((max_blk_nnz + 1) & ~1);
  return cap * (pair ? 16 : 8) + static_cast<size_t>(max_dict) * 16 + (state ? static_cast<size_t>(max_dict + (max_dict & 1)) * 8 : 0) +
         (RBA + 4) * 4 + (cap / 8 + 3) * 16;
}
size_t rowgather_smem_bytes(int max_blk_nnz, int max_dict) { return rowgather_lds_bytes(max_blk_nnz, max_dict, true, false); }
size_t ct_smem_bytes(int max_blk_nnz, int max_dict) { return rowgather_lds_bytes(max_blk_nnz, max_dict, true, true); }

template <class V, class... KArgs, class... Tail>
int launch_rowgather(hf_ctx* ctx,
                     void (*kernel)(int, int, int, const int32_t*, const int4*, const uint4*, const uint4*, const double2*, KArgs...),
                     const char* (*info)(), Tail... tail) {
  const int cap = (ctx->max_blk_nnz + 1) & ~1;
  const int capd = ctx->rg_max_dict;
  const size_t sm = rowgather_lds_bytes(ctx->max_blk_nnz, capd, V::PAIR, V::STATE);
  int& grid = ctx->rg_grid[V::ID];
  if (grid == 0) {
    const void* fn = reinterpret_cast<const void*>(kernel);
    if (sm > 64 * 1024) HF_HIP(hipFuncSetAttribute(fn, hipFuncAttributeMaxDynamicSharedMemorySize, static_cast<int>(sm)));
    int per_cu = 0, ncu = 0;
    HF_HIP(hipOccupancyMaxActiveBlocksPerMultiprocessor(&per_cu, fn, RBA, sm));
    HF_HIP(hipDeviceGetAttribute(&ncu, hipDeviceAttributeMultiprocessorCount, ctx->dev));
    grid = std::max(1, std::min(ctx->nblk_a, std::max(1, per_cu) * std::max(1, ncu)));
    if (const char* label = info ? info() : nullptr)
      std::fprintf(stderr, "%s: %zu bytes of dynamic LDS, %d workgroups per CU, grid %d of %d blocks\n", label, sm, per_cu, grid, ctx->nblk_a);
  }
  hipLaunchKernelGGL(kernel, dim3(grid), dim3(RBA), sm, ctx->stream, ctx->nblk_a, cap, capd, ctx->d_rowptr, ctx->d_rg_hdr,
                     reinterpret_cast<const uint4*>(ctx->d_rg_ell), reinterpret_cast<const uint4*>(ctx->d_rg_cid), ctx->d_rg_zrb,
                     static_cast<KArgs>(tail)...);
  HF_HIP(hipGetLastError());
  return HF_OK;
}

template <bool KONLY = false>
int launch_assemble_rows(hf_ctx* ctx, const double* kappa_idx, const double* rhoc_idx, double dt, double* Mout, double* Aout) {
  return launch_rowgather<RowsConst<KONLY>>(ctx, &k_assemble_rows<KONLY>, nullptr, kappa_idx, rhoc_idx, dt, Mout, Aout);
}

template <bool KONLY = false>
int launch_assemble_rows_an(hf_ctx* ctx, const double* kappa_idx, const double* rhoc_idx, double dt, double* Mout, double* Aout) {
  const auto info = []() -> const char* {
    const char* e = std::getenv("HEATFLOW_ANISO_INFO");
    return e && e[0] == '1' ? (KONLY ? "[aniso] k_assemble_rows_an<true>" : "[aniso] k_assemble_rows_an<false>") : nullptr;
  };
  return launch_rowgather<RowsAniso<KONLY>>(ctx, &k_assemble_rows_an<KONLY>, info, kappa_idx, rhoc_idx, ctx->an.d_m, dt, Mout, Aout);
}

template <bool KONLY = false>
int launch_assemble_rows_any(hf_ctx* ctx, const double* kappa_idx, const double* rhoc_idx, double dt, double* Mout, double* Aout) {
  if (ctx->an.on) return launch_assemble_rows_an<KONLY>(ctx, kappa_idx, rhoc_idx, dt, Mout, Aout);
  return launch_assemble_rows<KONLY>(ctx, kappa_idx, rhoc_idx, dt, Mout, Aout);
}

int launch_assemble(hf_ctx* ctx) {
  if (ctx->mode == HF_ASM_ROW_GATHER && ctx->rg_ok)
    return launch_assemble_rows_any(ctx, ctx->d_kappa_rg, ctx->d_rhoc_rg, ctx->dt, ctx->d_M, ctx->d_A);
  if (ctx->mode == HF_ASM_ROW_GATHER)
    return launch_assemble_lds(ctx, true, ctx->d_kappa, ctx->d_rhoc, ctx->dt, ctx->d_M, ctx->d_A);
  if (ctx->mode == HF_ASM_LDS_COLORED || ctx->mode == HF_ASM_LDS_ATOMIC) {
    return launch_assemble_lds(ctx, ctx->mode == HF_ASM_LDS_COLORED, ctx->d_kappa, ctx->d_rhoc, ctx->dt, ctx->d_M, ctx->d_A);
  } else {
    HF_HIP(hipMemsetAsync(ctx->d_M, 0, sizeof(double) * ctx->nnz, ctx->stream));
    HF_HIP(hipMemsetAsync(ctx->d_A, 0, sizeof(double) * ctx->nnz, ctx->stream));
    hipLaunchKernelGGL(k_assemble_global, dim3((ctx->ne + TPB - 1) / TPB), dim3(TPB), 0, ctx->stream, ctx->ne,
                       ctx->d_rowptr, ctx->d_colidx, ctx->d_elem, ctx->d_zr, ctx->d_kappa, ctx->d_rhoc, ctx->dt,
                       ctx->d_M, ctx->d_A);
  }
  HF_HIP(hipGetLastError());
  return HF_OK;
}

template <int MODE, typename VT = double>
void launch_spmv(hf_ctx* c, const VT* vals, const double* x, double* y, double* part0 = nullptr,
                 const double* bvec = nullptr, double* pvec = nullptr, double* part1 = nullptr,
                 double* part2 = nullptr, double w = 0.0, const double* dinv = nullptr, hipEvent_t ev_start = nullptr,
                 hipEvent_t ev_stop = nullptr, int parity = 0) {
  const ColComp comp{c->d_cdict_ptr, c->d_cdict, c->d_cid, c->max_chunk_nnz_s, c->cdict_own ? 1 : 0};
#define HF_SPMV_ARGS c->n, c->nchunks_s, static_cast<int>(SRPC), static_cast<const int32_t*>(c->d_rowptr),                    \
                     static_cast<const int32_t*>(c->d_colidx), vals, x, y, (MODE == 0 ? nullptr : c->d_scal), part0, bvec,  \
                     dinv ? dinv : static_cast<const double*>(c->d_dinv), pvec, part1, part2, w, c->P, parity, comp
  const std::uint32_t smem = static_cast<std::uint32_t>(spmv_smem_bytes(c));
  if (c->c16) {
    if (ev_start != nullptr) hipExtLaunchKernelGGL((k_spmv<MODE, true, VT, HF_SPMV_UN>), dim3(c->Ps), dim3(TS), smem, c->stream, ev_start, ev_stop, 0u, HF_SPMV_ARGS);
    else hipLaunchKernelGGL((k_spmv<MODE, true, VT, HF_SPMV_UN>), dim3(c->Ps), dim3(TS), smem, c->stream, HF_SPMV_ARGS);
  } else {
    if (ev_start != nullptr) hipExtLaunchKernelGGL((k_spmv<MODE, false, VT>), dim3(c->Ps), dim3(TS), smem, c->stream, ev_start, ev_stop, 0u, HF_SPMV_ARGS);
    else hipLaunchKernelGGL((k_spmv<MODE, false, VT>), dim3(c->Ps), dim3(TS), smem, c->stream, HF_SPMV_ARGS);
  }
#undef HF_SPMV_ARGS
}

constexpr int PROF_PAIRS = 64;

struct LinSys { const double* A; const double* dinv; double* x; const double* b; };

void launch_pcg_iteration(hf_ctx* c, const LinSys& s, int parity) {
  const bool timed = c->prof && c->prof_used < PROF_PAIRS;
  hipEvent_t e0 = timed ? c->prof_ev[2 * c->prof_used] : nullptr, e1 = timed ? c->prof_ev[2 * c->prof_used + 1] : nullptr;
  launch_spmv<9>(c, s.A, c->d_z, c->d_Ap, c->d_part_pAp, nullptr, c->d_p, c->d_part_rz, c->d_part_zz, 0.0, nullptr, e0, e1,
                 parity);
  if (timed) c->prof_used++;
  hipLaunchKernelGGL(k_pcg_update, dim3(c->P), dim3(TPB), 0, c->stream, c->n, c->nchunks, c->P, parity, c->d_scal,
                     c->d_part_pAp, c->d_part_rz, c->d_part_zz, s.x, c->d_r, c->d_p, c->d_Ap, s.dinv, c->d_z);
}

}
```

heatflow_amd/csrc/hf_solver.hpp:

```cpp
#pragma once
#include "hf_pattern.hpp"

namespace {

using DevCsr = hf_ctx::DevCsr;
using DevLevel = hf_ctx::DevLevel;

void free_dev_csr(DevCsr& m) { dev_free(&m.ptr); dev_free(&m.idx); dev_free(&m.val); dev_free(&m.valf); dev_free(&m.dptr); dev_free(&m.dict); dev_free(&m.cid); m = DevCsr(); }

void free_amg(hf_ctx* ctx) {
  for (size_t l = 0; l < ctx->amg.size(); ++l) {
    DevLevel& L = ctx->amg[l];
    if (l > 0) { free_dev_csr(L.A); dev_free(&L.dinv); dev_free(&L.x); dev_free(&L.cat); }
    if (L.own_b) dev_free(&L.b);
    free_dev_csr(L.P); free_dev_csr(L.R); free_dev_csr(L.Rt); free_dev_csr(L.GP);
  }
  ctx->amg.clear();
  dev_free(&ctx->d_coarse_inv);
  dev_free(&ctx->d_coarse_inv_f);
  ctx->coarse_n = 0;
  ctx->amg_ready = false;
}

int lanes_for_avg(double avg) {
// ... 584 lines not shown
  ctx->resp_solves += 1;
  *w_out = w;
  if (ctx->start_kind == 3 && ctx->proj.ready) {
    const int slot = PROJ_MH + static_cast<int>(ctx->resp.size());
    HF_TRY(proj_store(ctx, slot, w, ctx->d_b));
    proj_column(ctx, slot, nullptr, false);
  }
  return HF_OK;
}

int prepare_response(hf_ctx* ctx, const double* g_new, int max_it, RespArgs* ra) {
  const int nb = ctx->nbc;
  ra->k = 0;
  std::vector<double> rem(nb);
  double nrm2 = 0.0, gn2 = 0.0;
  for (int q = 0; q < nb; ++q) {
    rem[q] = (g_new[q] - ctx->h_g0[q]) - (ctx->h_g0[q] - ctx->h_g1[q]);
    nrm2 += rem[q] * rem[q];
    gn2 += g_new[q] * g_new[q];
  }
  if (!(nrm2 > 0.0)) return HF_OK;
  for (size_t k = 0; k < ctx->resp.size(); ++k) {
    const std::vector<double>& d = ctx->resp[k].dir;
    double c = 0.0;
    for (int q = 0; q < nb; ++q) c += d[q] * rem[q];
    for (int q = 0; q < nb; ++q) rem[q] -= c * d[q];
    ra->c[k] = c;
    ra->w[k] = ctx->resp[k].w;
  }
  double rn2 = 0.0;
  for (int q = 0; q < nb; ++q) rn2 += rem[q] * rem[q];
  if (rn2 > 1e-12 * nrm2 && nrm2 > 1e-18 * gn2 && ctx->resp.size() < static_cast<size_t>(MAXRESP)) {
    const double rn = std::sqrt(rn2);
    hf_ctx::BcResponse nr;
    nr.dir.resize(nb);
    for (int q = 0; q < nb; ++q) nr.dir[q] = rem[q] / rn;
    const int rc = solve_response(ctx, nr.dir, max_it, &nr.w);
    if (rc == HF_ERR_HIP) return rc;
    if (rc == HF_OK) {
      ra->c[ctx->resp.size()] = rn;
      ra->w[ctx->resp.size()] = nr.w;
      ctx->resp.push_back(std::move(nr));
    } else {
      ctx->start_kind = 1;
    }
  }
  ra->k = static_cast<int>(ctx->resp.size());
  return HF_OK;
}

void launch_rhs(hf_ctx* ctx) {
  if (ctx->have_load)
    launch_spmv<10>(ctx, ctx->d_M, ctx->d_u, ctx->d_b, nullptr, nullptr, nullptr, nullptr, nullptr, ctx->dt, ctx->d_load);
  else
    launch_spmv<0>(ctx, ctx->d_M, ctx->d_u, ctx->d_b);
}

void launch_rhs_bdf2(hf_ctx* ctx, bool extrap) {
  const double* um1 = ctx->bdf_hist ? ctx->d_uprev : ctx->d_u;
  if (ctx->have_load) {
    if (extrap) launch_spmv<15>(ctx, ctx->d_M, ctx->d_u, ctx->d_b, nullptr, um1, ctx->d_ustart, nullptr, nullptr, ctx->dt, ctx->d_load);
    else launch_spmv<14>(ctx, ctx->d_M, ctx->d_u, ctx->d_b, nullptr, um1, ctx->d_ustart, nullptr, nullptr, ctx->dt, ctx->d_load);
  } else {
    if (extrap) launch_spmv<13>(ctx, ctx->d_M, ctx->d_u, ctx->d_b, nullptr, um1, ctx->d_ustart);
    else launch_spmv<12>(ctx, ctx->d_M, ctx->d_u, ctx->d_b, nullptr, um1, ctx->d_ustart);
  }
}

int kt_finish(hf_ctx* ctx) {
  if (ctx->nbc > 0) {
    if (ctx->nlift > 0)
      hipLaunchKernelGGL(k_take_lift, dim3((ctx->nlift + 255) / 256), dim3(256), 0, ctx->stream, ctx->nlift, ctx->d_lift_slot, ctx->d_A,
                         ctx->d_lift_val);
    hipLaunchKernelGGL(k_bc_rows, dim3((ctx->nbc + 255) / 256), dim3(256), 0, ctx->stream, ctx->nbc, ctx->d_bc_dofs, ctx->d_rowptr,
                       ctx->d_colidx, ctx->d_A);
  }
  hipLaunchKernelGGL(k_dinv, dim3((ctx->n + 255) / 256), dim3(256), 0, ctx->stream, ctx->n, ctx->d_rowptr, ctx->d_colidx, ctx->d_A,
                     ctx->d_dinv);
  HF_HIP(hipGetLastError());
  return HF_OK;
}

int kt_revalue(hf_ctx* ctx, const double* u, const double* uprev) {
  if (ctx->kt.c_on)
    HF_TRY(launch_rowgather<RowsBothT>(ctx, &k_assemble_rows_cT, nullptr, ctx->d_rg_dict, ctx->kt.hdr, ctx->kt.vals, ctx->kt.chdr,
                                       ctx->kt.cvals, ctx->d_kappa_rg, ctx->d_rhoc_rg, ctx->dt, u, uprev, ctx->d_M, ctx->d_A));
  else
    HF_TRY(launch_rowgather<RowsKappaT>(ctx, &k_assemble_rows_kT, nullptr, ctx->d_rg_dict, ctx->kt.hdr, ctx->kt.vals,
                                        ctx->d_kappa_rg, ctx->d_rhoc_rg, ctx->dt, u, uprev, ctx->d_A));
  return kt_finish(ctx);
}

int steady_revalue(hf_ctx* ctx, const KTab* hdr, const double* u, double* Kout) {
  const auto info = []() -> const char* { return std::getenv("HEATFLOW_DEBUG") ? "[steady picard] k_assemble_rows_kT_K" : nullptr; };
  return launch_rowgather<RowsKappaTK>(ctx, &k_assemble_rows_kT_K, info, ctx->d_rg_dict, hdr, ctx->kt.vals, ctx->d_kappa_rg, u, Kout);
}

int step_solve(hf_ctx* ctx, double rtol, double atol, int max_it) {
  const LinSys sys{ctx->d_A, ctx->d_dinv, ctx->d_u, ctx->d_b};
  const bool use_amg = ctx->precond == 1 && ctx->amg_ready;
  int rc = pcg_solve(ctx, sys, use_amg, rtol, atol, max_it, &ctx->pred_iters);
  if (rc == HF_ERR_NOCONV && use_amg && ctx->h_scal->done == 2) {
    ctx->amg_fallbacks += 1;
    int pred = 0;
    rc = pcg_solve(ctx, sys, false, rtol, atol, max_it, &pred);
  }
  return rc;
}

int step_device(hf_ctx* ctx, const double* g_host, const double* g_dev, double rtol, double atol, int max_it, bool last = true) {
  const int nb = ctx->nbc;
  RespArgs ra{};
  ra.k = 0;
  const bool kt = ctx->kt.on;
  const int kind = kt && ctx->start_kind >= 2 ? 1 : ctx->start_kind;
  const bool projected = kind == 3;
  const bool bdf2 = ctx->scheme == HF_TIME_BDF2;
  if (projected) HF_TRY(proj_ensure(ctx));
  const bool hist_ok = nb > 0 && ctx->extrapolate && ctx->have_prev && ctx->g_hist >= 2;
  if (kind >= 2 && hist_ok && !(bdf2 && kind == 2)) HF_TRY(prepare_response(ctx, g_host, max_it, &ra));
  const int sweeps = kt ? ctx->kt.picard : 1;
  const bool ct = kt && ctx->kt.c_on;
  const bool track = kt && last;
  if (kt) {
    const double* um1 = bdf2 && ctx->bdf_hist ? ctx->d_uprev : nullptr;
    HF_TRY(kt_revalue(ctx, ctx->d_u, um1));
    if (ctx->precond == 1 && ctx->amg_ready) ctx->amg_fine_stale = true;
    if (track && sweeps == 1)
      hipLaunchKernelGGL(k_eval_state, dim3(ctx->P), dim3(TPB), 0, ctx->stream, ctx->n, ctx->d_u, um1, ctx->kt.pic);
    if (ct && sweeps > 1)
      hipLaunchKernelGGL(k_picard_w, dim3(ctx->P), dim3(TPB), 0, ctx->stream, ctx->n, ctx->d_u,
                         bdf2 ? (ctx->bdf_hist ? ctx->d_uprev : ctx->d_u) : nullptr, ctx->kt.w);
  }
  const double* g = g_dev ? g_dev : ctx->d_g;
  if (nb > 0 && !g_dev) HF_HIP(hipMemcpyAsync(ctx->d_g, g_host, sizeof(double) * nb, hipMemcpyHostToDevice, ctx->stream));
  if (bdf2 && (projected || !ctx->extrapolate)) {
    launch_rhs_bdf2(ctx, false);
    std::swap(ctx->d_uprev, ctx->d_ustart);
    ctx->bdf_hist = true;
    ctx->have_prev = true;
  } else if (bdf2) {
    launch_rhs_bdf2(ctx, true);
    HF_HIP(hipMemcpyAsync(ctx->d_uprev, ctx->d_u, sizeof(double) * ctx->n, hipMemcpyDeviceToDevice, ctx->stream));
    HF_HIP(hipMemcpyAsync(ctx->d_u, ctx->d_ustart, sizeof(double) * ctx->n, hipMemcpyDeviceToDevice, ctx->stream));
    ctx->bdf_hist = true;
    ctx->have_prev = true;
  } else if (projected) {
    launch_rhs(ctx);
    ctx->have_prev = true;
  } else if (ctx->extrapolate && ctx->have_prev) {
    if (ctx->have_load)
      launch_spmv<11>(ctx, ctx->d_M, ctx->d_u, ctx->d_b, nullptr, ctx->d_uprev, ctx->d_ustart, nullptr, nullptr, ctx->dt, ctx->d_load);
    else
      launch_spmv<8>(ctx, ctx->d_M, ctx->d_u, ctx->d_b, nullptr, ctx->d_uprev, ctx->d_ustart);
    HF_HIP(hipMemcpyAsync(ctx->d_uprev, ctx->d_u, sizeof(double) * ctx->n, hipMemcpyDeviceToDevice, ctx->stream));
    if (ra.k > 0)
      hipLaunchKernelGGL(k_start_vector, dim3(ctx->P), dim3(TPB), 0, ctx->stream, ctx->n, ctx->d_ustart, ra, ctx->d_u);
    else
      HF_HIP(hipMemcpyAsync(ctx->d_u, ctx->d_ustart, sizeof(double) * ctx->n, hipMemcpyDeviceToDevice, ctx->stream));
  } else {
    launch_rhs(ctx);
    if (ctx->extrapolate) {
      HF_HIP(hipMemcpyAsync(ctx->d_uprev, ctx->d_u, sizeof(double) * ctx->n, hipMemcpyDeviceToDevice, ctx->stream));
      ctx->have_prev = true;
    }
  }
// ... 113 lines not shown
```

heatflow_amd/hip_backend.py:

```python
from __future__ import annotations

import ctypes as C
import os
import subprocess

import numpy as np

_HERE = os.path.dirname(os.path.abspath(__file__))
LIB_PATH = os.environ.get("HEATFLOW_HIP_LIB") or os.path.join(_HERE, "csrc", "libheatflow_hip.so")

HF_OK, HF_ERR_ARG, HF_ERR_STATE, HF_ERR_HIP, HF_ERR_NOCONV, HF_ERR_ALLOC = 0, -1, -2, -3, -4, -5
ASM_LDS_ATOMIC, ASM_LDS_COLORED, ASM_GLOBAL_ATOMIC, ASM_ROW_GATHER = 0, 1, 2, 3
PC_JACOBI, PC_AMG = 0, 1
K_SPMV, K_PCG_SPMV, K_PCG_UPDATE, K_PCG_DIR, K_ASSEMBLE, K_RHS, K_STREAM_READ = range(7)
BATCH_SHARED, BATCH_PER_COLUMN, BATCH_AFFINE = 0, 1, 2
TIME_BACKWARD_EULER, TIME_BDF2 = 0, 1
TIME_SCHEMES = {"backward_euler": TIME_BACKWARD_EULER, "bdf2": TIME_BDF2}


def time_scheme_code(name):
    if name not in TIME_SCHEMES:
        raise ValueError(f"unknown time scheme {name!r} (expected one of {sorted(TIME_SCHEMES)})")
    return TIME_SCHEMES[name]

EXPORTS = [
    "hf_version", "hf_create", "hf_destroy", "hf_last_error", "hf_set_mesh", "hf_set_mesh_prebuilt", "hf_pattern_export_size",
    "hf_pattern_export", "hf_amg_export_size", "hf_amg_export", "hf_amg_install", "hf_set_materials",
    "hf_update_kappa", "hf_set_dirichlet", "hf_assemble", "hf_set_time_scheme", "hf_set_precond", "hf_set_start_vector", "hf_get_response_solves", "hf_get_amg_info", "hf_get_amg_fallbacks", "hf_set_state", "hf_get_state", "hf_sample", "hf_step", "hf_run",
    "hf_batch_begin", "hf_batch_load_column", "hf_batch_set_affine", "hf_batch_set_state", "hf_batch_get_state", "hf_batch_run", "hf_batch_run_flux", "hf_batch_end",
    "hf_flux_setup", "hf_flux_project", "hf_flux_solve", "hf_flux_sample",
    "hf_steady_setup", "hf_steady_solve", "hf_steady_picard_setup", "hf_steady_picard_solve", "hf_set_load", "hf_get_load", "hf_hold_load",
    "hf_tangent_setup", "hf_run_tangent", "hf_get_tangent", "hf_set_kappa_tables", "hf_get_picard_change", "hf_set_rhoc_tables", "hf_set_picard", "hf_set_anisotropy", "hf_get_sizes", "hf_get_csr", "hf_spmv",
    "hf_amg_apply", "hf_batch_apply_precond", "hf_dense_inverse", "hf_time_kernel", "hf_set_profile", "hf_get_profile", "hf_last_gpu_ms",
]


class HipUnavailable(RuntimeError):
    """libheatflow_hip.so is not built or no HIP device is usable."""


class HipError(RuntimeError):
    def __init__(self, code, msg):
        super().__init__(f"heatflow_hip error {code}: {msg}")
        self.code = code


class NotConverged(HipError):
    pass


def build_library(force=False, verbose=False):
    src = os.path.join(_HERE, "csrc", "heatflow_hip.hip")
    hdr = os.path.join(_HERE, "..", "include", "heatflow_hip.h")
    if not force and os.path.isfile(LIB_PATH):
        csrc = os.path.join(_HERE, "csrc")
        newest = max([os.path.getmtime(src), os.path.getmtime(hdr)] +
                     [os.path.getmtime(os.path.join(csrc, f)) for f in os.listdir(csrc) if f.endswith(".hpp")])
        if os.path.getmtime(LIB_PATH) >= newest:
            return LIB_PATH
    cmd = ["make", "-C", os.path.join(_HERE, "csrc"), "libheatflow_hip.so"]
    if force:
        cmd.insert(1, "-B")
    res = subprocess.run(cmd, capture_output=True, text=True)
    if verbose or res.returncode != 0:
        print(res.stdout, res.stderr)
    if res.returncode != 0:
        raise RuntimeError("building libheatflow_hip.so failed:\n" + res.stderr)
    return LIB_PATH


_lib = None


def load_library():
    global _lib
    if _lib is not None:
        return _lib
    if not os.path.isfile(LIB_PATH):
        raise HipUnavailable(f"{LIB_PATH} not found - run `python -c 'import __graft_entry__ as g; g.build()'` "
                             "or `make -C heatflow_amd/csrc`")
    lib = C.CDLL(LIB_PATH)
    vp, i32, i64, dbl = C.c_void_p, C.c_int32, C.c_int64, C.c_double
    pd, pi = C.POINTER(C.c_double), C.POINTER(C.c_int32)
    lib.hf_version.restype = C.c_char_p
    lib.hf_last_error.restype = C.c_char_p
    lib.hf_last_error.argtypes = [vp]
    protos = {
        "hf_create": [C.c_int, C.POINTER(vp)],
        "hf_destroy": [vp],
        "hf_set_mesh": [vp, i32, i32, pd, pi, pi],
        "hf_set_mesh_prebuilt": [vp, i32, i32, pd, pi, pi, vp, i64],
        "hf_pattern_export_size": [vp, C.POINTER(i64)],
        "hf_pattern_export": [vp, vp, i64],
        "hf_amg_export_size": [vp, C.POINTER(i64)],
        "hf_amg_export": [vp, vp, i64],
        "hf_amg_install": [vp, vp, i64],
        "hf_set_materials": [vp, i32, pi, pd, pd],
        "hf_update_kappa": [vp, i32, pi, pd],
        "hf_set_dirichlet": [vp, i32, pi],
        "hf_assemble": [vp, dbl, i32],
        "hf_set_time_scheme": [vp, i32],
        "hf_set_precond": [vp, i32, i32],
        "hf_set_start_vector": [vp, i32],
        "hf_get_response_solves": [vp, C.POINTER(i64)],
        "hf_get_amg_info": [vp, pi, pi, i32, pd, pd],
        "hf_get_amg_fallbacks": [vp, C.POINTER(i64)],
        "hf_set_state": [vp, pd],
        "hf_get_state": [vp, pd],
        "hf_sample": [vp, i32, pi, pd],
        "hf_step": [vp, pd, dbl, dbl, i32, pi, pd],
        "hf_run": [vp, i32, pd, dbl, dbl, i32, i32, pi, pd, pi],
        "hf_batch_begin": [vp, i32, i32],
        "hf_batch_load_column": [vp, i32],
        "hf_batch_set_affine": [vp, i32, pi, pd],
        "hf_batch_set_state": [vp, i32, pd],
        "hf_batch_get_state": [vp, i32, pd],
        "hf_batch_run": [vp, i32, pd, dbl, dbl, i32, i32, pi, pd, pi],
        "hf_batch_run_flux": [vp, i32, pd, dbl, dbl, i32, i32, pi, pd, pi, i32, dbl, i32, i32, pi, pd, pi],
        "hf_batch_end": [vp],
        "hf_flux_setup": [vp],
        "hf_flux_project": [vp, dbl, i32, pd, pd, pi],
        "hf_flux_solve": [vp, i32, dbl, i32, pi],
        "hf_flux_sample": [vp, i32, pi, pd, pd],
        "hf_steady_setup": [vp, i32, pi, i32],
        "hf_steady_solve": [vp, pd, i32, dbl, dbl, i32, pi, pd],
        "hf_steady_picard_setup": [vp, i32, pi, i32],
        "hf_steady_picard_solve": [vp, pd, i32, dbl, dbl, i32, dbl, i32, pi, pi, pd, pd],
        "hf_set_load": [vp, pd],
        "hf_get_load": [vp, pd],
        "hf_hold_load": [vp],
        "hf_tangent_setup": [vp, i32, pi],
        "hf_run_tangent": [vp, i32, pd, pd, dbl, dbl, i32, i32, pi, pd, pi, pd, pi],
        "hf_get_tangent": [vp, i32, pd],
        "hf_set_kappa_tables": [vp, i32, pi, pd, pd, pi, pd, i32],
        "hf_get_picard_change": [vp, pd],
        "hf_set_rhoc_tables": [vp, i32, pi, pd, pd, pi, pd],
        "hf_set_picard": [vp, i32],
        "hf_set_anisotropy": [vp, i32, pi, pd, pd],
        "hf_get_sizes": [vp, pi, pi, C.POINTER(i64), pi],
        "hf_get_csr": [vp, pi, pi, pd, pd],
        "hf_spmv": [vp, i32, pd, pd],
        "hf_amg_apply": [vp, pd, pd, pd],
        "hf_batch_apply_precond": [vp, pd, pd, pd],
        "hf_dense_inverse": [vp, i32, pi, pi, pd, pd, pd, pd, pd],
        "hf_time_kernel": [vp, i32, i32, pd],
        "hf_last_gpu_ms": [vp, pd],
        "hf_set_profile": [vp, i32],
        "hf_get_profile": [vp, pd, C.POINTER(i64)],
    }
    for name, args in protos.items():
        fn = getattr(lib, name)
        fn.argtypes = args
        fn.restype = C.c_int
    _lib = lib
    return lib


def blob_address(blob):
    if isinstance(blob, tuple):
        return int(blob[0]), int(blob[1]), blob
    if hasattr(blob, "address") and hasattr(blob, "nbytes") and not isinstance(blob, np.ndarray):
        return int(blob.address), int(blob.nbytes), blob
    arr = np.ascontiguousarray(blob, dtype=np.uint8)
    return arr.ctypes.data, arr.nbytes, arr


def _pd(a):
    return a.ctypes.data_as(C.POINTER(C.c_double)) if a is not None else None


def _pi(a):
    return a.ctypes.data_as(C.POINTER(C.c_int32)) if a is not None else None


def _f64(a):
    return np.ascontiguousarray(a, dtype=np.float64)


def _i32(a):
    return np.ascontiguousarray(a, dtype=np.int32)


class HeatflowHIP:

    def __init__(self, device_id=0):
        self._lib = load_library()
        self._ctx = C.c_void_p()
        rc = self._lib.hf_create(int(device_id), C.byref(self._ctx))
        if rc != HF_OK:
            msg = self._lib.hf_last_error(self._ctx).decode() if self._ctx else "no usable HIP device"
            if self._ctx:
                self._lib.hf_destroy(self._ctx)
                self._ctx = C.c_void_p()
            raise HipUnavailable(f"hf_create(device {device_id}) failed ({rc}): {msg}")
        self.n = self.n_e = self.n_bc = 0
        self.nnz = 0
        self.batch_nv = 0

    def close(self):
        if getattr(self, "_ctx", None):
            self._lib.hf_destroy(self._ctx)
            self._ctx = C.c_void_p()

    def __del__(self):
        try:
            self.close()
        except Exception:
            pass

    def __enter__(self):
        return self

    def __exit__(self, *exc):
        self.close()

    def _check(self, rc):
        if rc == HF_OK:
            return
        msg = self._lib.hf_last_error(self._ctx).decode()
        if rc == HF_ERR_NOCONV:
            raise NotConverged(rc, msg)
        if rc == HF_ERR_ARG:
            raise ValueError(f"heatflow_hip: {msg}")
        raise HipError(rc, msg)
# ... 287 lines not shown
        self._check(self._lib.hf_flux_project(self._ctx, rtol, int(max_it), _pd(gz), _pd(gr), _pi(it)))
        self.last_flux_iters = it
        return gz, gr

    def flux_solve(self, rtol=1e-10, max_it=5000, want_z=True, want_r=True):
        it = np.zeros(2, dtype=np.int32)
        self._check(self._lib.hf_flux_solve(self._ctx, (1 if want_z else 0) | (2 if want_r else 0), rtol, int(max_it), _pi(it)))
        self.last_flux_iters = it
        return it

    def flux_sample(self, nodes, want_z=True, want_r=True):
        nodes = np.ascontiguousarray(nodes, dtype=np.int32)
        gz = np.empty(len(nodes), dtype=np.float64) if want_z else None
        gr = np.empty(len(nodes), dtype=np.float64) if want_r else None
        self._check(self._lib.hf_flux_sample(self._ctx, len(nodes), _pi(nodes), _pd(gz), _pd(gr)))
        return gz, gr

    def steady_setup(self, dofs, precond=PC_JACOBI):
        d = _i32(dofs)
        self._check(self._lib.hf_steady_setup(self._ctx, len(d), _pi(d) if len(d) else None, int(precond)))
        self.n_steady = len(d)

    def steady_solve(self, g, use_load=False, rtol=1e-10, atol=0.0, max_it=20000):
        g = _f64(g)
        if g.shape != (getattr(self, "n_steady", -1),):
            raise ValueError(f"steady_solve: expected {getattr(self, 'n_steady', 0)} boundary values (steady_setup first)")
        it, res = C.c_int32(), C.c_double()
        rc = self._lib.hf_steady_solve(self._ctx, _pd(g), 1 if use_load else 0, rtol, atol, int(max_it), C.byref(it), C.byref(res))
        self.last_iters, self.last_resid = it.value, res.value
        self._check(rc)
        return it.value, res.value

    def steady_picard_setup(self, dofs, precond=PC_JACOBI):
        d = _i32(dofs)
        self._check(self._lib.hf_steady_picard_setup(self._ctx, len(d), _pi(d) if len(d) else None, int(precond)))
        self.n_steady = len(d)

    def steady_picard_solve(self, g, use_load=False, rtol=1e-10, atol=0.0, max_it=20000, picard_tol=1e-6, max_sweeps=50):
        g = _f64(g)
        if g.shape != (getattr(self, "n_steady", -1),):
            raise ValueError(f"steady_picard_solve: expected {getattr(self, 'n_steady', 0)} boundary values (steady_picard_setup first)")
        ms = int(max_sweeps)
        sw, chg, nl = C.c_int32(), C.c_double(), C.c_double()
        its = np.zeros(max(ms, 1), dtype=np.int32)
        rc = self._lib.hf_steady_picard_solve(self._ctx, _pd(g), 1 if use_load else 0, rtol, atol, int(max_it), float(picard_tol), ms,
                                              C.byref(sw), _pi(its), C.byref(chg), C.byref(nl))
        info = {"sweeps": sw.value, "iters": [int(v) for v in its[:sw.value]], "change": chg.value, "nl_resid": nl.value}
        self.last_picard = info
        self.last_iters, self.last_resid = sum(info["iters"]), nl.value
        self._check(rc)
        return info

    def set_load(self, F):
        if F is None:
            self._check(self._lib.hf_set_load(self._ctx, None))
            return
        F = _f64(F)
        if F.shape != (self.n,):
            raise ValueError(f"set_load: expected {self.n} values")
        self._check(self._lib.hf_set_load(self._ctx, _pd(F)))

    def hold_load(self):
        self._check(self._lib.hf_hold_load(self._ctx))

    def get_load(self):
        F = np.empty(self.n, dtype=np.float64)
        self._check(self._lib.hf_get_load(self._ctx, _pd(F)))
        return F

    def get_csr(self, values=True):
        rowptr = np.empty(self.n + 1, dtype=np.int32)
        colidx = np.empty(self.nnz, dtype=np.int32)
        A = np.empty(self.nnz, dtype=np.float64) if values else None
        M = np.empty(self.nnz, dtype=np.float64) if values else None
        self._check(self._lib.hf_get_csr(self._ctx, _pi(rowptr), _pi(colidx), _pd(A), _pd(M)))
        return rowptr, colidx, A, M

    def spmv(self, x, which=0):
        x = _f64(x)
        y = np.empty(self.n, dtype=np.float64)
        self._check(self._lib.hf_spmv(self._ctx, int(which), _pd(x), _pd(y)))
        return y

    def amg_apply(self, r):
        r = _f64(r)
        if r.shape != (self.n,):
            raise ValueError(f"amg_apply: vector of {self.n} entries expected")
        z = np.empty(self.n, dtype=np.float64)
        rz = C.c_double()
        self._check(self._lib.hf_amg_apply(self._ctx, _pd(r), _pd(z), C.byref(rz)))
        return z, rz.value

    def batch_apply_precond(self, R):
        R = _f64(R)
        if R.shape != (self.batch_nv, self.n):
            raise ValueError(f"batch_apply_precond: array of shape ({self.batch_nv}, {self.n}) expected")
        Z = np.empty_like(R)
        rz = np.empty(self.batch_nv, dtype=np.float64)
        self._check(self._lib.hf_batch_apply_precond(self._ctx, _pd(R), _pd(Z), _pd(rz)))
        return Z, rz

    def dense_inverse(self, S, b):
        S = S.tocsr()
        S.sort_indices()
        n = S.shape[0]
        ptr, idx, val, b = _i32(S.indptr), _i32(S.indices), _f64(S.data), _f64(b)
        inv = np.empty((n, n), dtype=np.float64)
        x64 = np.empty(n, dtype=np.float64)
        x32 = np.empty(n, dtype=np.float64)
        self._check(self._lib.hf_dense_inverse(self._ctx, int(n), _pi(ptr), _pi(idx), _pd(val), _pd(b), _pd(inv), _pd(x64), _pd(x32)))
        return inv, x64, x32

    def time_kernel(self, which, reps=50):
        ms = C.c_double()
        self._check(self._lib.hf_time_kernel(self._ctx, int(which), int(reps), C.byref(ms)))
        return ms.value

    def set_profile(self, on=True):
        self._check(self._lib.hf_set_profile(self._ctx, 1 if on else 0))

    def get_profile(self):
        ms, cnt = C.c_double(), C.c_int64()
        self._check(self._lib.hf_get_profile(self._ctx, C.byref(ms), C.byref(cnt)))
        return ms.value, cnt.value

    def last_gpu_ms(self):
        ms = C.c_double()
        self._check(self._lib.hf_last_gpu_ms(self._ctx, C.byref(ms)))
        return ms.value

    @staticmethod
    def version():
        return load_library().hf_version().decode()
```

include/heatflow_hip.h:

```cpp
#ifndef HEATFLOW_HIP_H
#define HEATFLOW_HIP_H

#include <stdint.h>

#ifdef __cplusplus
extern "C" {
#endif

typedef struct hf_ctx hf_ctx;

enum {
  HF_OK = 0,
  HF_ERR_ARG = -1,
  HF_ERR_STATE = -2,
  HF_ERR_HIP = -3,
  HF_ERR_NOCONV = -4,
  HF_ERR_ALLOC = -5
};

enum { HF_ASM_LDS_ATOMIC = 0, HF_ASM_LDS_COLORED = 1, HF_ASM_GLOBAL_ATOMIC = 2, HF_ASM_ROW_GATHER = 3 };

enum {
  HF_K_SPMV = 0,
  HF_K_PCG_SPMV = 1,
// ... 19 lines not shown

int hf_set_materials(hf_ctx* ctx, int32_t n_mat, const int32_t* tags, const double* kappa, const double* rho_c);

int hf_update_kappa(hf_ctx* ctx, int32_t n_mat, const int32_t* tags, const double* kappa);

int hf_set_anisotropy(hf_ctx* ctx, int32_t n, const int32_t* tags, const double* m_z, const double* m_r);

int hf_set_dirichlet(hf_ctx* ctx, int32_t n_bc, const int32_t* dofs);

int hf_assemble(hf_ctx* ctx, double dt, int32_t mode);

enum { HF_TIME_BACKWARD_EULER = 0, HF_TIME_BDF2 = 1 };
int hf_set_time_scheme(hf_ctx* ctx, int32_t scheme);

int hf_set_precond(hf_ctx* ctx, int32_t kind, int32_t reuse);
int hf_get_amg_info(hf_ctx* ctx, int32_t* n_levels, int32_t* level_rows, int32_t max_levels, double* op_complexity,
                    double* setup_seconds);

int hf_amg_export_size(hf_ctx* ctx, int64_t* bytes);
int hf_amg_export(hf_ctx* ctx, void* blob, int64_t bytes);
int hf_amg_install(hf_ctx* ctx, const void* blob, int64_t bytes);

int hf_set_start_vector(hf_ctx* ctx, int32_t kind);
int hf_get_response_solves(hf_ctx* ctx, int64_t* count);

int hf_get_amg_fallbacks(hf_ctx* ctx, int64_t* count);

int hf_set_state(hf_ctx* ctx, const double* u);
int hf_get_state(hf_ctx* ctx, double* u);
int hf_sample(hf_ctx* ctx, int32_t n_s, const int32_t* nodes, double* out);

int hf_step(hf_ctx* ctx, const double* g_bc, double rtol, double atol, int32_t max_it, int32_t* iters, double* resid);

int hf_run(hf_ctx* ctx, int32_t n_steps, const double* g_bc_all, double rtol, double atol, int32_t max_it,
           int32_t n_s, const int32_t* nodes, double* samples, int32_t* iters);

enum { HF_BATCH_SHARED = 0, HF_BATCH_PER_COLUMN = 1, HF_BATCH_AFFINE = 2 };
int hf_batch_begin(hf_ctx* ctx, int32_t nv, int32_t operator_kind);
int hf_batch_load_column(hf_ctx* ctx, int32_t j);
int hf_batch_set_affine(hf_ctx* ctx, int32_t n_tags, const int32_t* tags, const double* delta );
int hf_batch_set_state(hf_ctx* ctx, int32_t j, const double* u);
int hf_batch_get_state(hf_ctx* ctx, int32_t j, double* u);
int hf_batch_run(hf_ctx* ctx, int32_t n_steps, const double* g_bc_all, double rtol, double atol, int32_t max_it,
                 int32_t n_s, const int32_t* nodes, double* samples, int32_t* iters);
int hf_batch_run_flux(hf_ctx* ctx, int32_t n_steps, const double* g_bc_all, double rtol, double atol, int32_t max_it,
                      int32_t n_s, const int32_t* nodes, double* samples, int32_t* iters, int32_t flux_components,
                      double flux_rtol, int32_t flux_max_it, int32_t n_fs, const int32_t* flux_nodes, double* flux_samples,
                      int32_t* flux_iters);
int hf_batch_end(hf_ctx* ctx);

int hf_flux_setup(hf_ctx* ctx);
int hf_flux_project(hf_ctx* ctx, double rtol, int32_t max_it, double* grad_z, double* grad_r, int32_t* iters);
int hf_flux_solve(hf_ctx* ctx, int32_t components, double rtol, int32_t max_it, int32_t* iters);
int hf_flux_sample(hf_ctx* ctx, int32_t n_s, const int32_t* nodes, double* grad_z, double* grad_r);

int hf_steady_setup(hf_ctx* ctx, int32_t n_s, const int32_t* dofs_s, int32_t precond);
int hf_steady_solve(hf_ctx* ctx, const double* g_s, int32_t use_load, double rtol, double atol, int32_t max_it, int32_t* iters,
                    double* resid);

int hf_steady_picard_setup(hf_ctx* ctx, int32_t n_s, const int32_t* dofs_s, int32_t precond);
int hf_steady_picard_solve(hf_ctx* ctx, const double* g_s, int32_t use_load, double rtol, double atol, int32_t max_it,
                           double picard_tol, int32_t max_sweeps, int32_t* sweeps, int32_t* iters, double* change, double* nl_resid);
int hf_set_load(hf_ctx* ctx, const double* F);
int hf_hold_load(hf_ctx* ctx);
int hf_get_load(hf_ctx* ctx, double* F);

int hf_tangent_setup(hf_ctx* ctx, int32_t n_par, const int32_t* tag_col);
int hf_run_tangent(hf_ctx* ctx, int32_t n_steps, const double* g_all, const double* h_all, double rtol, double atol, int32_t max_it,
                   int32_t n_s, const int32_t* nodes, double* samples, int32_t* iters, double* tangent_samples, int32_t* tangent_iters);
int hf_get_tangent(hf_ctx* ctx, int32_t j, double* s);

int hf_set_kappa_tables(hf_ctx* ctx, int32_t n_tab, const int32_t* tags, const double* t0, const double* dT, const int32_t* n_knots,
                        const double* values, int32_t picard_sweeps);
int hf_get_picard_change(hf_ctx* ctx, double* max_du);

int hf_set_rhoc_tables(hf_ctx* ctx, int32_t n_tab, const int32_t* tags, const double* t0, const double* dT, const int32_t* n_knots,
                       const double* values);
int hf_set_picard(hf_ctx* ctx, int32_t sweeps);

int hf_get_sizes(hf_ctx* ctx, int32_t* n, int32_t* n_e, int64_t* nnz, int32_t* n_bc);
int hf_get_csr(hf_ctx* ctx, int32_t* rowptr, int32_t* colidx, double* A, double* M);
int hf_spmv(hf_ctx* ctx, int32_t which, const double* x, double* y);

int hf_amg_apply(hf_ctx* ctx, const double* r, double* z, double* rz);
int hf_batch_apply_precond(hf_ctx* ctx, const double* r, double* z, double* rz);
int hf_dense_inverse(hf_ctx* ctx, int32_t n, const int32_t* ptr, const int32_t* idx, const double* val, const double* b,
                     double* inv, double* x64, double* x32);

int hf_time_kernel(hf_ctx* ctx, int32_t which, int32_t reps, double* ms_avg);
int hf_set_profile(hf_ctx* ctx, int32_t on);
int hf_get_profile(hf_ctx* ctx, double* spmv_ms_sum, int64_t* spmv_launches);
int hf_last_gpu_ms(hf_ctx* ctx, double* ms);

#ifdef __cplusplus
}
#endif
#endif
```

Before: 721.9 million.

## Compress SpMV matrix values into per-chunk deduplicated value lists

```diff
diff --git a/heatflow_amd/csrc/heatflow_hip.hip b/heatflow_amd/csrc/heatflow_hip.hip
--- a/heatflow_amd/csrc/heatflow_hip.hip
+++ b/heatflow_amd/csrc/heatflow_hip.hip
@@ -89,6 +89,7 @@
   tangent_free(ctx);
   kt_free(ctx);
   an_free(ctx);
+  value_lists_free(ctx);
   ctx->n = n; ctx->ne = ne; ctx->nnz = static_cast<int64_t>(T.colidx.size());
   ctx->nchunks = (n + RB - 1) / RB;
   ctx->nblk_a = (n + RBA - 1) / RBA;
@@ -546,6 +547,7 @@
   if (device_id < 0 || device_id >= count) return HF_ERR_ARG;
   hf_ctx* ctx = new hf_ctx();
   ctx->dev = device_id;
+  if (const char* e = std::getenv("HEATFLOW_VALUE_LISTS")) ctx->vl_mode = (e[0] == '0') ? 0 : (e[0] == '2') ? 2 : 1;
   auto bail = [&](int rc) { *out = ctx; return rc; };
   if (hipSetDevice(device_id) != hipSuccess) return bail(fail(ctx, HF_ERR_HIP, "hipSetDevice(%d) failed", device_id));
   if (hipStreamCreateWithFlags(&ctx->stream, hipStreamNonBlocking) != hipSuccess)
@@ -583,7 +585,7 @@
   dev_free(&ctx->d_uprev); dev_free(&ctx->d_ustart);
   dev_free(&ctx->d_u); dev_free(&ctx->d_b); dev_free(&ctx->d_r); dev_free(&ctx->d_p); dev_free(&ctx->d_Ap);
   free_batch(ctx); free_batch_state(ctx->fluxb); free_batch_cols(ctx); free_amg(ctx); free_responses(ctx); proj_free(ctx); dev_free(&ctx->d_z); dev_free(&ctx->d_z2);
-  steady_free(ctx); load_free(ctx); tangent_free(ctx); kt_free(ctx); an_free(ctx);
+  steady_free(ctx); load_free(ctx); tangent_free(ctx); kt_free(ctx); an_free(ctx); value_lists_free(ctx);
   dev_free(&ctx->d_M1); dev_free(&ctx->d_dinv1); dev_free(&ctx->d_gz); dev_free(&ctx->d_gr); dev_free(&ctx->d_bz); dev_free(&ctx->d_br);
   dev_free(&ctx->d_tmp); dev_free(&ctx->d_part_pAp); dev_free(&ctx->d_part_rz); dev_free(&ctx->d_part_zz);
   dev_free(&ctx->d_part_bn); dev_free(&ctx->d_scal); dev_free(&ctx->d_samp_idx); dev_free(&ctx->d_samp); dev_free(&ctx->d_fsamp_idx);
@@ -799,6 +801,8 @@
   ctx->dt = ctx->scheme == HF_TIME_BDF2 ? 2.0 * dt / 3.0 : dt;
   ctx->mode = mode;
   HF_HIP(hipEventRecord(ctx->ev0, ctx->stream));
+  value_lists_touch(ctx, ctx->d_A);
+  value_lists_touch(ctx, ctx->d_M);
   HF_TRY(launch_assemble(ctx));
   if (ctx->kt.on) {
     HF_TRY(kt_revalue(ctx, ctx->d_u, nullptr));
@@ -813,12 +817,18 @@
     hipLaunchKernelGGL(k_dinv, dim3((ctx->n + 255) / 256), dim3(256), 0, ctx->stream, ctx->n, ctx->d_rowptr,
                        ctx->d_colidx, ctx->d_A, ctx->d_dinv);
   }
+  const bool lists = value_lists_wanted(ctx);
+  if (lists) {
+    HF_TRY(value_lists_build(ctx, 0, ctx->d_A));
+    HF_TRY(value_lists_build(ctx, 1, ctx->d_M));
+  }
   HF_HIP(hipEventRecord(ctx->ev1, ctx->stream));
   HF_HIP(hipGetLastError());
   HF_HIP(hipStreamSynchronize(ctx->stream));
   float ms = 0.f;
   HF_HIP(hipEventElapsedTime(&ms, ctx->ev0, ctx->ev1));
   ctx->last_ms = ms;
+  if (lists) HF_TRY(value_lists_finish(ctx));
   if (ctx->precond == 1) {
     OperatorPrint now;
     HF_TRY(operator_print(ctx, now));
@@ -1422,6 +1432,7 @@
 }
 
 int steady_eliminate(hf_ctx* ctx) {
+  value_lists_touch(ctx, ctx->d_A);
   HF_HIP(hipMemcpyAsync(ctx->d_A, ctx->steady.Kfree, sizeof(double) * ctx->nnz, hipMemcpyDeviceToDevice, ctx->stream));
   if (ctx->nlift > 0)
     hipLaunchKernelGGL(k_take_lift, dim3((ctx->nlift + 255) / 256), dim3(256), 0, ctx->stream, ctx->nlift, ctx->d_lift_slot,
@@ -1929,6 +1940,34 @@
   return HF_OK;
 }
 
+int hf_set_value_lists(hf_ctx* ctx, int32_t mode) {
+  if (!ctx) return HF_ERR_ARG;
+  if (mode < 0 || mode > 2) return fail(ctx, HF_ERR_ARG, "hf_set_value_lists: unknown mode %d", mode);
+  ctx->vl_mode = mode;
+  return HF_OK;
+}
+
+int hf_get_value_lists(hf_ctx* ctx, int32_t which, int32_t* valid, int64_t* sum_vlist, int32_t* max_vlist, int32_t* vcap, int32_t* vptr,
+                       double* vlist, uint32_t* cv) {
+  if (!ctx) return HF_ERR_ARG;
+  if (which < 0 || which > 1) return fail(ctx, HF_ERR_ARG, "hf_get_value_lists: which = %d (0 = A, 1 = M)", which);
+  if (!ctx->assembled) return fail(ctx, HF_ERR_STATE, "hf_get_value_lists before hf_assemble");
+  const hf_ctx::ValueLists& L = ctx->vl[which];
+  const bool live = L.valid && L.src == (which ? ctx->d_M : ctx->d_A);
+  if (valid) *valid = live ? 1 : 0;
+  if (sum_vlist) *sum_vlist = L.sum_vlist;
+  if (max_vlist) *max_vlist = L.max_vlist;
+  if (vcap) *vcap = ctx->vl_vcap;
+  if (vptr || vlist || cv) {
+    if (!live) return fail(ctx, HF_ERR_STATE, "hf_get_value_lists: the tables of %s are not valid", which ? "M" : "A");
+    HF_HIP(hipSetDevice(ctx->dev));
+    if (vptr) HF_HIP(copy_sync(ctx, vptr, L.vptr, sizeof(int32_t) * (static_cast<size_t>(ctx->nchunks_s) + 1), hipMemcpyDeviceToHost));
+    if (vlist) HF_HIP(copy_sync(ctx, vlist, L.vlist, sizeof(double) * static_cast<size_t>(L.sum_vlist), hipMemcpyDeviceToHost));
+    if (cv) HF_HIP(copy_sync(ctx, cv, L.cv, sizeof(uint32_t) * static_cast<size_t>(ctx->nnz), hipMemcpyDeviceToHost));
+  }
+  return HF_OK;
+}
+
 int hf_spmv(hf_ctx* ctx, int32_t which, const double* x, double* y) {
   if (!ctx) return HF_ERR_ARG;
   if (!ctx->assembled || !x || !y || which < 0 || which > 1) return fail(ctx, HF_ERR_STATE, "hf_spmv: not assembled or bad arguments");
diff --git a/heatflow_amd/csrc/hf_context.hpp b/heatflow_amd/csrc/hf_context.hpp
--- a/heatflow_amd/csrc/hf_context.hpp
+++ b/heatflow_amd/csrc/hf_context.hpp
@@ -104,6 +104,19 @@
   int max_cdict = 0;
   bool cdict_own = false;
   bool c16 = true;
+  struct ValueLists {
+    const double* src = nullptr;
+    int32_t *vptr = nullptr, *count = nullptr, *info = nullptr;
+    double* vlist = nullptr;
+    uint32_t* cv = nullptr;
+    int64_t cap = 0;
+    int64_t sum_vlist = 0;
+    int max_vlist = 0;
+    bool valid = false;
+  } vl[2];
+  int vl_mode = 1;
+  int vl_vcap = 0;
+  int vl_occ = 0;
   bool have_mesh = false, have_mat = false, assembled = false;
   double dt = 0.0;
   double dt_step = 0.0;
diff --git a/heatflow_amd/csrc/hf_kernels.hpp b/heatflow_amd/csrc/hf_kernels.hpp
--- a/heatflow_amd/csrc/hf_kernels.hpp
+++ b/heatflow_amd/csrc/hf_kernels.hpp
@@ -807,6 +807,7 @@
 }
 
 struct ColComp { const int32_t* dptr; const int32_t* dict; const uint16_t* id; int xd_off; int own; };
+struct ValComp : ColComp { const int32_t* vptr; const double* vlist; const uint32_t* cv; int vl_off; int vcap; };
 
 #ifndef HF_NT_STREAM
 #define HF_NT_STREAM 0
@@ -841,7 +842,7 @@
 
 __device__ __forceinline__ double bdf2_operand(double un, double unm1) { return (4.0 * un - unm1) * (1.0 / 3.0); }
 
-template <int MODE, bool C16 = false, typename VT = double, int UN = 8>
+template <int MODE, bool C16 = false, typename VT = double, int UN = 8, bool VC = false>
 __global__ __launch_bounds__(TS) __attribute__((amdgpu_waves_per_eu(8, 8))) void k_spmv(int n, int nchunks, int rpc ,
                                               const int32_t* __restrict__ rowptr, const int32_t* __restrict__ colidx,
                                               const VT* __restrict__ vals, const double* __restrict__ x,
@@ -850,7 +851,7 @@
                                               const double* __restrict__ dinv, double* __restrict__ pvec,
                                               double* __restrict__ part1, double* __restrict__ part2, double w,
                                               int npart ,
-                                              int parity, ColComp comp) {
+                                              int parity, typename std::conditional<VC, ValComp, ColComp>::type comp) {
   extern __shared__ double sprod[];
   __shared__ double s4[TS / 64];
   __shared__ int s_own;
@@ -894,7 +895,8 @@
     }
     return conv;
   };
-  constexpr bool PIPELINED = C16 && (HF_PIPE == 2 || (HF_PIPE == 1 && sizeof(VT) == 4));
+  constexpr bool PIPELINED = C16 && !VC && (HF_PIPE == 2 || (HF_PIPE == 1 && sizeof(VT) == 4));
+  static_assert(!VC || (C16 && sizeof(VT) == 8), "value lists: the fine operator's f64 arrays on compressed columns");
   if (!PIPELINED && cycle_gate()) return;
   const ChunkIter sched(nchunks);
   HF_STAMP(0);
@@ -1084,7 +1086,68 @@
       pb = rowptr[prow + 1] - k0;
     }
     RowOps e = row_operands(min(prow, r1 - 1), C16 && comp.own != 0);
-    if (C16) {
+    if constexpr (VC) {
+      double* xd = sprod + comp.xd_off;
+      double* vl = sprod + comp.vl_off;
+      const int d0 = comp.dptr[chunk], nd = comp.dptr[chunk + 1] - d0;
+      const int v0 = comp.vptr[chunk], nv = comp.vptr[chunk + 1] - v0;
+      const bool vin = nv <= comp.vcap;
+      int k = k0 + threadIdx.x;
+      std::uint32_t cw[HF_UNROLL];
+#pragma unroll
+      for (int u = 0; u < HF_UNROLL; ++u) cw[u] = (k + u * TS < k1) ? stream_load(&comp.cv[k + u * TS]) : 0u;
+      double lv[2];
+#pragma unroll
+      for (int u = 0; u < 2; ++u) {
+        const int i = static_cast<int>(threadIdx.x) + u * TS;
+        lv[u] = (vin && i < nv) ? comp.vlist[v0 + i] : 0.0;
+      }
+      for (int i = threadIdx.x; i < nd; i += HF_STAGE_U * TS) {
+        int c[HF_STAGE_U];
+        double xv[HF_STAGE_U];
+#pragma unroll
+        for (int u = 0; u < HF_STAGE_U; ++u) c[u] = (i + u * TS < nd) ? comp.dict[d0 + i + u * TS] : 0;
+#pragma unroll
+        for (int u = 0; u < HF_STAGE_U; ++u) xv[u] = (i + u * TS < nd) ? opnd(c[u]) : 0.0;
+#pragma unroll
+        for (int u = 0; u < HF_STAGE_U; ++u)
+          if (i + u * TS < nd) {
+            xd[i + u * TS] = xv[u];
+            if ((MODE == 4 || MODE == 8 || MODE == 9 || MODE == 11) && c[u] == r0) s_own = i + u * TS;
+          }
+      }
+#pragma unroll
+      for (int u = 0; u < 2; ++u) {
+        const int i = static_cast<int>(threadIdx.x) + u * TS;
+        if (vin && i < nv) vl[i] = lv[u];
+      }
+      if (vin)
+        for (int i = threadIdx.x + 2 * TS; i < nv; i += TS) vl[i] = comp.vlist[v0 + i];
+      __syncthreads();
+      HF_STAMP(stamp_at); ++stamp_at;
+      if ((MODE == 4 || MODE == 8 || MODE == 9 || MODE == 11) && comp.own && pin) e.x = xd[s_own + (prow - r0)];
+      while (k < k1) {
+        const int kn = k + HF_UNROLL * TS;
+        std::uint32_t cn[HF_UNROLL];
+#pragma unroll
+        for (int u = 0; u < HF_UNROLL; ++u) cn[u] = (kn + u * TS < k1) ? stream_load(&comp.cv[kn + u * TS]) : 0u;
+        if (vin) {
+#pragma unroll
+          for (int u = 0; u < HF_UNROLL; ++u)
+            if (k + u * TS < k1) sprod[k - k0 + u * TS] = vl[cw[u] >> 16] * xd[cw[u] & 0xffffu];
+        } else {
+          double gv[HF_UNROLL];
+#pragma unroll
+          for (int u = 0; u < HF_UNROLL; ++u) gv[u] = (k + u * TS < k1) ? comp.vlist[v0 + static_cast<int>(cw[u] >> 16)] : 0.0;
+#pragma unroll
+          for (int u = 0; u < HF_UNROLL; ++u)
+            if (k + u * TS < k1) sprod[k - k0 + u * TS] = gv[u] * xd[cw[u] & 0xffffu];
+        }
+#pragma unroll
+        for (int u = 0; u < HF_UNROLL; ++u) cw[u] = cn[u];
+        k = kn;
+      }
+    } else if (C16) {
       double* xd = sprod + comp.xd_off;
       const int d0 = comp.dptr[chunk], nd = comp.dptr[chunk + 1] - d0;
       int k = k0 + threadIdx.x;
@@ -1169,6 +1232,119 @@
       part2[blockIdx.x] = t2;
       for (int q = blockIdx.x + gridDim.x; q < npart; q += gridDim.x) { part1[q] = 0.0; part2[q] = 0.0; }
     }
+  }
+}
+
+constexpr int VL_MAX_CHUNK = 4096;
+
+template <int NW>
+__device__ __forceinline__ int block_scan_incl(int v, int* sw, int& total) {
+  const int lane = threadIdx.x & 63, w = threadIdx.x >> 6;
+#pragma unroll
+  for (int o = 1; o < 64; o <<= 1) {
+    const int t = __shfl_up(v, o, 64);
+    if (lane >= o) v += t;
+  }
+  if (lane == 63) sw[w] = v;
+  __syncthreads();
+  int before = 0;
+  total = 0;
+#pragma unroll
+  for (int q = 0; q < NW; ++q) {
+    const int t = sw[q];
+    if (q < w) before += t;
+    total += t;
+  }
+  __syncthreads();
+  return v + before;
+}
+
+__global__ __launch_bounds__(TS) void k_vl_ids(int n, int nchunks, int rpc, const int32_t* __restrict__ rowptr,
+                                               const double* __restrict__ vals, const uint16_t* __restrict__ cid,
+                                               std::uint32_t* __restrict__ cv, int32_t* __restrict__ count) {
+  __shared__ unsigned long long skey[VL_MAX_CHUNK];
+  __shared__ uint16_t sorg[VL_MAX_CHUNK];
+  __shared__ int sw[TS / 64];
+  const int tid = static_cast<int>(threadIdx.x);
+  for (int chunk = blockIdx.x; chunk < nchunks; chunk += gridDim.x) {
+    const int r0 = chunk * rpc, r1 = min(n, r0 + rpc);
+    const int k0 = rowptr[r0], m = min(rowptr[r1] - k0, VL_MAX_CHUNK);
+    int np = 64;
+    while (np < m) np <<= 1;
+    for (int i = tid; i < np; i += TS) {
+      skey[i] = i < m ? static_cast<unsigned long long>(__double_as_longlong(vals[k0 + i])) : ~0ull;
+      sorg[i] = static_cast<uint16_t>(i);
+    }
+    __syncthreads();
+    for (int size = 2; size <= np; size <<= 1)
+      for (int stride = size >> 1; stride > 0; stride >>= 1) {
+        for (int t = tid; t < (np >> 1); t += TS) {
+          const int lo = 2 * t - (t & (stride - 1)), hi = lo + stride;
+          const bool up = (lo & size) == 0;
+          const unsigned long long ka = skey[lo], kb = skey[hi];
+          const uint16_t oa = sorg[lo], ob = sorg[hi];
+          const bool gt = ka > kb || (ka == kb && oa > ob);
+          if (gt == up) { skey[lo] = kb; skey[hi] = ka; sorg[lo] = ob; sorg[hi] = oa; }
+        }
+        __syncthreads();
+      }
+    const int per = (np + TS - 1) / TS;
+    const int i0 = tid * per;
+    int heads = 0;
+    for (int j = 0; j < per; ++j) {
+      const int i = i0 + j;
+      if (i < m && (i == 0 || skey[i] != skey[i - 1])) ++heads;
+    }
+    int total = 0;
+    int run = block_scan_incl<TS / 64>(heads, sw, total) - heads;
+    for (int j = 0; j < per; ++j) {
+      const int i = i0 + j;
+      if (i < m) {
+        if (i == 0 || skey[i] != skey[i - 1]) ++run;
+        const int k = k0 + sorg[i];
+        cv[k] = static_cast<std::uint32_t>(cid[k]) | (static_cast<std::uint32_t>(run - 1) << 16);
+      }
+    }
+    if (tid == 0) count[chunk] = total;
+    __syncthreads();
+  }
+}
+
+__global__ __launch_bounds__(1024) void k_vl_scan(int nchunks, const int32_t* __restrict__ count, int32_t* __restrict__ vptr,
+                                                  int32_t* __restrict__ info) {
+  __shared__ int sw[16];
+  __shared__ int smax[16];
+  const int tid = static_cast<int>(threadIdx.x);
+  int carry = 0, mx = 0;
+  for (int base = 0; base < nchunks; base += 1024) {
+    const int i = base + tid;
+    const int v = i < nchunks ? count[i] : 0;
+    mx = max(mx, v);
+    int total = 0;
+    const int incl = block_scan_incl<16>(v, sw, total);
+    if (i < nchunks) vptr[i] = carry + incl - v;
+    carry += total;
+  }
+#pragma unroll
+  for (int o = 32; o > 0; o >>= 1) mx = max(mx, __shfl_down(mx, o, 64));
+  if ((tid & 63) == 0) smax[tid >> 6] = mx;
+  __syncthreads();
+  if (tid == 0) {
+    for (int q = 1; q < 16; ++q) mx = max(mx, smax[q]);
+    vptr[nchunks] = carry;
+    info[0] = carry;
+    info[1] = mx;
+  }
+}
+
+__global__ __launch_bounds__(TS) void k_vl_lists(int n, int nchunks, int rpc, const int32_t* __restrict__ rowptr,
+                                                 const double* __restrict__ vals, const std::uint32_t* __restrict__ cv,
+                                                 const int32_t* __restrict__ vptr, long long cap, double* __restrict__ vlist) {
+  if (vptr[nchunks] > cap) return;
+  for (int chunk = blockIdx.x; chunk < nchunks; chunk += gridDim.x) {
+    const int r0 = chunk * rpc, r1 = min(n, r0 + rpc);
+    const int k0 = rowptr[r0], k1 = rowptr[r1], v0 = vptr[chunk];
+    for (int k = k0 + threadIdx.x; k < k1; k += TS) vlist[v0 + static_cast<int>(cv[k] >> 16)] = vals[k];
   }
 }
 
diff --git a/heatflow_amd/csrc/hf_pattern.hpp b/heatflow_amd/csrc/hf_pattern.hpp
--- a/heatflow_amd/csrc/hf_pattern.hpp
+++ b/heatflow_amd/csrc/hf_pattern.hpp
@@ -396,6 +396,99 @@
   return HF_OK;
 }
 
+inline void value_lists_touch(hf_ctx* c, const double* vals) {
+  for (auto& L : c->vl)
+    if (L.src == vals) L.valid = false;
+}
+inline const hf_ctx::ValueLists* value_lists_of(const hf_ctx* c, const double* vals) {
+  for (const auto& L : c->vl)
+    if (L.valid && L.src == vals) return &L;
+  return nullptr;
+}
+inline const hf_ctx::ValueLists* value_lists_of(const hf_ctx*, const float*) { return nullptr; }
+
+void value_lists_free(hf_ctx* ctx) {
+  for (auto& L : ctx->vl) {
+    dev_free(&L.vptr); dev_free(&L.count); dev_free(&L.info); dev_free(&L.vlist); dev_free(&L.cv);
+    L = hf_ctx::ValueLists();
+  }
+  ctx->vl_vcap = 0; ctx->vl_occ = 0;
+}
+
+bool value_lists_wanted(const hf_ctx* ctx) {
+  return ctx->vl_mode != 0 && ctx->c16 && !ctx->kt.on && ctx->max_chunk_nnz_s <= VL_MAX_CHUNK && ctx->nchunks_s > 0;
+}
+
+int value_lists_build(hf_ctx* ctx, int which, const double* vals) {
+  hf_ctx::ValueLists& L = ctx->vl[which];
+  L.valid = false;
+  L.src = vals;
+  const int64_t want = ctx->vl_mode == 2 ? ctx->nnz : ctx->nnz / 2;
+  if (!L.cv) {
+    HF_TRY(dev_alloc(ctx, &L.cv, ctx->nnz));
+    HF_TRY(dev_alloc(ctx, &L.vptr, static_cast<size_t>(ctx->nchunks_s) + 1));
+    HF_TRY(dev_alloc(ctx, &L.count, ctx->nchunks_s));
+    HF_TRY(dev_alloc(ctx, &L.info, 2));
+  }
+  if (!L.vlist || L.cap < want) {
+    HF_TRY(dev_alloc(ctx, &L.vlist, std::max<int64_t>(want, 1)));
+    L.cap = want;
+  }
+  const int grid = std::min(ctx->nchunks_s, 4096);
+  hipLaunchKernelGGL(k_vl_ids, dim3(grid), dim3(TS), 0, ctx->stream, ctx->n, ctx->nchunks_s, static_cast<int>(SRPC), ctx->d_rowptr, vals,
+                     ctx->d_cid, L.cv, L.count);
+  hipLaunchKernelGGL(k_vl_scan, dim3(1), dim3(1024), 0, ctx->stream, ctx->nchunks_s, L.count, L.vptr, L.info);
+  hipLaunchKernelGGL(k_vl_lists, dim3(grid), dim3(TS), 0, ctx->stream, ctx->n, ctx->nchunks_s, static_cast<int>(SRPC), ctx->d_rowptr, vals,
+                     L.cv, L.vptr, static_cast<long long>(L.cap), L.vlist);
+  HF_HIP(hipGetLastError());
+  return HF_OK;
+}
+
+int value_lists_vcap(hf_ctx* ctx, int longest) {
+  const void* fn = reinterpret_cast<const void*>(&k_spmv<9, true, double, HF_SPMV_UN, true>);
+  const size_t base = spmv_smem_bytes(ctx);
+  const int room = base < 64 * 1024 ? static_cast<int>((64 * 1024 - base) / 8) : 0;
+  int occ0 = 0;
+  HF_HIP(hipOccupancyMaxActiveBlocksPerMultiprocessor(&occ0, fn, TS, base));
+  int lo = 0, hi = std::min(longest, room), occ = occ0;
+  if (const char* e = std::getenv("HEATFLOW_VALUE_LISTS_VCAP")) {
+    lo = std::max(0, std::min(std::atoi(e), room));
+    HF_HIP(hipOccupancyMaxActiveBlocksPerMultiprocessor(&occ, fn, TS, base + static_cast<size_t>(lo) * 8));
+  } else {
+    while (lo < hi) {
+      const int mid = (lo + hi + 1) / 2;
+      int o = 0;
+      HF_HIP(hipOccupancyMaxActiveBlocksPerMultiprocessor(&o, fn, TS, base + static_cast<size_t>(mid) * 8));
+      if (o >= occ0) lo = mid; else hi = mid - 1;
+    }
+  }
+  ctx->vl_vcap = lo;
+  ctx->vl_occ = occ;
+  return HF_OK;
+}
+
+int value_lists_finish(hf_ctx* ctx) {
+  int longest = 0;
+  for (auto& L : ctx->vl) {
+    if (!L.src || !L.info) continue;
+    int32_t info[2] = {0, 0};
+    HF_HIP(copy_sync(ctx, info, L.info, sizeof info, hipMemcpyDeviceToHost));
+    L.sum_vlist = info[0];
+    L.max_vlist = info[1];
+    L.valid = L.sum_vlist <= L.cap && (ctx->vl_mode == 2 || L.sum_vlist <= ctx->nnz / 2);
+    if (L.valid) longest = std::max(longest, L.max_vlist);
+  }
+  if (longest > 0) HF_TRY(value_lists_vcap(ctx, longest));
+  if (std::getenv("HEATFLOW_DEBUG"))
+    for (int w = 0; w < 2; ++w)
+      std::fprintf(stderr, "[value lists] %s: %lld list entries for %lld nonzeros (share %.4f, %.2f bytes per nonzero), longest list %d, %s; %d entries per chunk in LDS, %d workgroups per CU\n",
+                   w ? "M" : "A", static_cast<long long>(ctx->vl[w].sum_vlist), static_cast<long long>(ctx->nnz),
+                   static_cast<double>(ctx->vl[w].sum_vlist) / static_cast<double>(std::max<int64_t>(ctx->nnz, 1)),
+                   4.0 + 8.0 * static_cast<double>(ctx->vl[w].sum_vlist) / static_cast<double>(std::max<int64_t>(ctx->nnz, 1)),
+                   ctx->vl[w].max_vlist, ctx->vl[w].valid ? "in use" : "not used", ctx->vl_vcap, ctx->vl_occ);
+  return HF_OK;
+}
+
 template <int MODE, typename VT = double>
 void launch_spmv(hf_ctx* c, const VT* vals, const double* x, double* y, double* part0 = nullptr,
                  const double* bvec = nullptr, double* pvec = nullptr, double* part1 = nullptr,
@@ -406,7 +499,19 @@
                      static_cast<const int32_t*>(c->d_colidx), vals, x, y, (MODE == 0 ? nullptr : c->d_scal), part0, bvec,  \
                      dinv ? dinv : static_cast<const double*>(c->d_dinv), pvec, part1, part2, w, c->P, parity, comp
   const std::uint32_t smem = static_cast<std::uint32_t>(spmv_smem_bytes(c));
-  if (c->c16) {
+  const hf_ctx::ValueLists* L = c->c16 ? value_lists_of(c, vals) : nullptr;
+  if (L != nullptr) {
+    if constexpr (std::is_same<VT, double>::value) {
+      const ValComp vcomp{comp, L->vptr, L->vlist, L->cv, c->max_chunk_nnz_s + c->max_cdict, c->vl_vcap};
+      const std::uint32_t smem_v = smem + static_cast<std::uint32_t>(c->vl_vcap) * 8u;
+#define HF_SPMV_VARGS c->n, c->nchunks_s, static_cast<int>(SRPC), static_cast<const int32_t*>(c->d_rowptr),                   \
+                      static_cast<const int32_t*>(c->d_colidx), vals, x, y, (MODE == 0 ? nullptr : c->d_scal), part0, bvec,  \
+                      dinv ? dinv : static_cast<const double*>(c->d_dinv), pvec, part1, part2, w, c->P, parity, vcomp
+      if (ev_start != nullptr) hipExtLaunchKernelGGL((k_spmv<MODE, true, double, HF_SPMV_UN, true>), dim3(c->Ps), dim3(TS), smem_v, c->stream, ev_start, ev_stop, 0u, HF_SPMV_VARGS);
+      else hipLaunchKernelGGL((k_spmv<MODE, true, double, HF_SPMV_UN, true>), dim3(c->Ps), dim3(TS), smem_v, c->stream, HF_SPMV_VARGS);
+#undef HF_SPMV_VARGS
+    }
+  } else if (c->c16) {
     if (ev_start != nullptr) hipExtLaunchKernelGGL((k_spmv<MODE, true, VT, HF_SPMV_UN>), dim3(c->Ps), dim3(TS), smem, c->stream, ev_start, ev_stop, 0u, HF_SPMV_ARGS);
     else hipLaunchKernelGGL((k_spmv<MODE, true, VT, HF_SPMV_UN>), dim3(c->Ps), dim3(TS), smem, c->stream, HF_SPMV_ARGS);
   } else {
diff --git a/heatflow_amd/csrc/hf_solver.hpp b/heatflow_amd/csrc/hf_solver.hpp
--- a/heatflow_amd/csrc/hf_solver.hpp
+++ b/heatflow_amd/csrc/hf_solver.hpp
@@ -690,6 +690,8 @@
 }
 
 int kt_revalue(hf_ctx* ctx, const double* u, const double* uprev) {
+  value_lists_touch(ctx, ctx->d_A);
+  if (ctx->kt.c_on) value_lists_touch(ctx, ctx->d_M);
   if (ctx->kt.c_on)
     HF_TRY(launch_rowgather<RowsBothT>(ctx, &k_assemble_rows_cT, nullptr, ctx->d_rg_dict, ctx->kt.hdr, ctx->kt.vals, ctx->kt.chdr,
                                        ctx->kt.cvals, ctx->d_kappa_rg, ctx->d_rhoc_rg, ctx->dt, u, uprev, ctx->d_M, ctx->d_A));
diff --git a/heatflow_amd/hip_backend.py b/heatflow_amd/hip_backend.py
--- a/heatflow_amd/hip_backend.py
+++ b/heatflow_amd/hip_backend.py
@@ -31,6 +31,7 @@
     "hf_flux_setup", "hf_flux_project", "hf_flux_solve", "hf_flux_sample",
     "hf_steady_setup", "hf_steady_solve", "hf_steady_picard_setup", "hf_steady_picard_solve", "hf_set_load", "hf_get_load", "hf_hold_load",
     "hf_tangent_setup", "hf_run_tangent", "hf_get_tangent", "hf_set_kappa_tables", "hf_get_picard_change", "hf_set_rhoc_tables", "hf_set_picard", "hf_set_anisotropy", "hf_get_sizes", "hf_get_csr", "hf_spmv",
+    "hf_set_value_lists", "hf_get_value_lists",
     "hf_amg_apply", "hf_batch_apply_precond", "hf_dense_inverse", "hf_time_kernel", "hf_set_profile", "hf_get_profile", "hf_last_gpu_ms",
 ]
 
@@ -140,6 +141,8 @@
         "hf_get_sizes": [vp, pi, pi, C.POINTER(i64), pi],
         "hf_get_csr": [vp, pi, pi, pd, pd],
         "hf_spmv": [vp, i32, pd, pd],
+        "hf_set_value_lists": [vp, i32],
+        "hf_get_value_lists": [vp, i32, pi, C.POINTER(i64), pi, pi, pi, pd, C.POINTER(C.c_uint32)],
         "hf_amg_apply": [vp, pd, pd, pd],
         "hf_batch_apply_precond": [vp, pd, pd, pd],
         "hf_dense_inverse": [vp, i32, pi, pi, pd, pd, pd, pd, pd],
@@ -593,6 +596,23 @@
         self._check(self._lib.hf_spmv(self._ctx, int(which), _pd(x), _pd(y)))
         return y
 
+    def set_value_lists(self, mode):
+        self._check(self._lib.hf_set_value_lists(self._ctx, int(mode)))
+
+    def get_value_lists(self, which=0, arrays=False):
+        valid, mx, vcap, total = C.c_int32(), C.c_int32(), C.c_int32(), C.c_int64()
+        self._check(self._lib.hf_get_value_lists(self._ctx, int(which), C.byref(valid), C.byref(total), C.byref(mx), C.byref(vcap),
+                                                 None, None, None))
+        out = {"valid": bool(valid.value), "sum_vlist": total.value, "max_vlist": mx.value, "vcap": vcap.value}
+        if arrays:
+            vptr = np.empty((self.n + 511) // 512 + 1, dtype=np.int32)
+            vlist = np.empty(total.value, dtype=np.float64)
+            cv = np.empty(self.nnz, dtype=np.uint32)
+            self._check(self._lib.hf_get_value_lists(self._ctx, int(which), None, None, None, None, _pi(vptr), _pd(vlist),
+                                                     cv.ctypes.data_as(C.POINTER(C.c_uint32))))
+            out.update(vptr=vptr, vlist=vlist, cv=cv)
+        return out
+
     def amg_apply(self, r):
         r = _f64(r)
         if r.shape != (self.n,):
diff --git a/include/heatflow_hip.h b/include/heatflow_hip.h
--- a/include/heatflow_hip.h
+++ b/include/heatflow_hip.h
@@ -125,6 +125,10 @@
 int hf_get_csr(hf_ctx* ctx, int32_t* rowptr, int32_t* colidx, double* A, double* M);
 int hf_spmv(hf_ctx* ctx, int32_t which, const double* x, double* y);
 
+int hf_set_value_lists(hf_ctx* ctx, int32_t mode);
+int hf_get_value_lists(hf_ctx* ctx, int32_t which, int32_t* valid, int64_t* sum_vlist, int32_t* max_vlist, int32_t* vcap, int32_t* vptr,
+                       double* vlist, uint32_t* cv);
+
 int hf_amg_apply(hf_ctx* ctx, const double* r, double* z, double* rz);
 int hf_batch_apply_precond(hf_ctx* ctx, const double* r, double* z, double* rz);
 int hf_dense_inverse(hf_ctx* ctx, int32_t n, const int32_t* ptr, const int32_t* idx, const double* val, const double* b,
```

After: 795.8 million, median of 6. 1.1x the previous value.
